# proger/haloop

Measured on AMD Instinct MI355X. Metric: utterances/sec, LSTM-CTC training step (fwd + CTC loss + bwd + clip + AdamW), higher is better.
Workload: dtype bf16 (dense operands rounded to bf16, 1 MFMA per product, fp32 accumulate; fp32 state, CTC, optimizer and master weights); 1 GPU; LC-2x1024: conv(80->128,k5,s4) + 2-layer LSTM H=1024 + Linear(1024->32) + CTC, 80 frames x 80 mels, vocab 32, targets 5-10 symbols, dropout 0.2; batch_per_gpu=64, global_batch=64, frames=80, mels=80, parallelism=dp1, hip_graph=False, math=bf16

## Files before the change

haloop_amd/_lib.py:

```python
import ctypes as C
import os

_HERE = os.path.dirname(os.path.abspath(__file__))
LIB_PATH = os.path.join(_HERE, 'csrc', 'libhalo.so')

HALO_ABI_VERSION = 19
HALO_GEMM_RELU = 1
HALO_GEMM_GELU = 2
HALO_GEMM_ACCUM = 4
HALO_GEMM_GELU_ERF = 8
HALO_CTC_FULL_LATTICE = 1
HALO_CTC_FINITE_MIN = 2
HALO_CTC_NO_LEAD_BLANK_LOOP = 4
HALO_CTC_WRAP_SKIP = 8
HALO_STREAM_SUBSAMPLE = 1
HALO_STREAM_CLASSIFIER = 2
HALO_STREAM_LSTM_LAYER0 = 16
HALO_SUMSQ_PARTS = 1024
HALO_MATH_F32 = 0
HALO_MATH_BF16X3 = 1
HALO_MATH_BF16 = 2

_vp, _i, _l, _f, _u64, _u32, _sz = C.c_void_p, C.c_int, C.c_long, C.c_float, C.c_uint64, C.c_uint32, C.c_size_t

SIGNATURES = {
    'halo_abi_version': (_i, []),
    'halo_debug_read': (_i, [_vp, _sz, _i, _sz, _vp, _vp]),
    'halo_strerror': (C.c_char_p, [_i]),
    'halo_device_info': (_i, [_i, C.c_char_p, _i, C.POINTER(_i)]),
    'halo_set_math_mode': (_i, [_i]),
    'halo_get_math_mode': (_i, []),
    'halo_set_scratch': (_i, [_vp, _sz]),
    'halo_set_lstm_fusion': (_i, [_i]),
    'halo_dropout_fwd': (_i, [_vp, _vp, _sz, _f, _u64, _u32, _u32, _vp, _vp]),
    'halo_counter_inc': (_i, [_vp, _vp]),
    'halo_gemm_f32': (_i, [_i, _i, _i, _i, _i, _vp, _i, _vp, _i, _vp, _i, _vp, _vp, _i, _f, _u64, _u32, _u32, _vp, _vp]),
    'halo_split_image_bytes': (_sz, [_i, _i]),
    'halo_split_image': (_i, [_vp, _i, _i, _i, _i, _vp, _vp]),
    'halo_layernorm_image': (_i, [_vp, _vp, _vp, _vp, _vp, _i, _i, _f, _vp]),
    'halo_layernorm_bf16': (_i, [_vp, _vp, _vp, _vp, _vp, _vp, _i, _i, _f, _vp]),
    'halo_cast_bf16': (_i, [_vp, _vp, _sz, _vp]),
    'halo_gelu_bf16': (_i, [_vp, _vp, _sz, _i, _vp]),
    'halo_gelu_bwd_bf16': (_i, [_vp, _vp, _vp, _sz, _i, _vp]),
    'halo_gemm_tn_bf16_group': (_i, [_i, _vp, _vp, _vp, _vp, _vp, _vp, _i, _vp, _vp, _i, _vp]),
    'halo_gemm_tn_rows_supported': (_i, [_i, _vp, _vp, _i]),
    'halo_gemm_tn_rows_preferred': (_i, [_i, _vp, _vp, _i]),
    'halo_gemm_tn_rows_group': (_i, [_i, _vp, _vp, _vp, _vp, _vp, _vp, _i, _vp, _vp, _vp]),
    'halo_gelu_b16': (_i, [_vp, _vp, _sz, _i, _vp]),
    'halo_gelu_bwd_b16': (_i, [_vp, _vp, _vp, _sz, _i, _vp]),
    'halo_dx_alloc': (_i, [_sz, _vp, _vp]),
    'halo_dx_open': (_i, [_vp, _vp]),
    'halo_dx_close': (_i, [_vp]),
    'halo_dx_free': (_i, [_vp]),
    'halo_dx_push': (_i, [_vp, _sz, _sz, _i, _vp, _sz, _i, _i, _vp]),
    'halo_dx_signal': (_i, [_vp, _sz, _i, _i, _u32, _vp]),
    'halo_dx_wait': (_i, [_vp, _i, _i, _u32, _vp]),
    'halo_dx_reduce': (_i, [_vp, _vp, _sz, _i, _i, _f, _vp]),
    'halo_attention_fwd_b16': (_i, [_vp, _l, _l, _vp, _vp, _l, _l, _vp, _l, _l, _vp, _l, _l, _vp, _i, _i, _i, _i, _i, _i, _vp]),
    'halo_attention_bwd_b16': (_i, [_vp, _l, _l, _vp, _vp, _l, _l, _vp, _vp, _l, _l, _vp, _vp, _vp, _vp, _vp, _l, _l, _i, _i, _i, _i, _i, _i, _vp]),
    'halo_gemm_rows_supported': (_i, [_i, _i, _i]),
    'halo_gemm_rows': (_i, [_vp, _vp, _l, _vp, _i, _i, _i, _vp, _l, _vp, _l, _vp, _l, _vp]),
    'halo_gemm_rows_gelu': (_i, [_vp, _vp, _l, _vp, _i, _i, _i, _vp, _vp, _l, _i, _vp]),
    'halo_gemm_rows_ce_workspace_bytes': (_sz, [_i, _i]),
    'halo_gemm_rows_ce': (_i, [_vp, _vp, _l, _vp, _i, _i, _i, _vp, _l, _vp, _vp, _vp, _vp, _l, _vp]),
    'halo_cross_entropy_bwd_bf16': (_i, [_vp, _vp, _vp, _vp, _l, _i, _i, _l, _l, _vp]),
    'halo_gemm_split_ce_workspace_bytes': (_sz, [_i, _i]),
    'halo_gemm_split_ce': (_i, [_vp, _vp, _i, _i, _i, _vp, _i, _vp, _vp, _l, _vp, _vp, _vp, _vp]),
    'halo_image_pair': (_i, [_vp, _vp, _i, _i, _l, _l, _i, _vp, _vp, _vp]),
    'halo_cross_entropy_bwd_images': (_i, [_vp, _vp, _vp, _vp, _l, _i, _i, _l, _l, _vp, _vp, _vp]),
    'halo_gemm_split': (_i, [_vp, _vp, _i, _i, _i, _vp, _i, _vp, _vp, _i, _f, _u64, _u32, _u32, _vp, _vp]),
    'halo_gemm_split_residual': (_i, [_vp, _vp, _i, _i, _i, _vp, _i, _vp, _i, _vp, _vp, _i, _f, _u64, _u32, _u32, _vp, _vp]),
    'halo_image_pairs': (_i, [_i, _vp, _vp, _vp, _vp, _vp, _vp, _vp]),
    'halo_gemm_split_io': (_i, [_vp, _vp, _vp, _l, _vp, _i, _i, _i, _vp, _i, _vp, _vp, _l, _vp, _i, _vp, _vp, _i, _vp]),
    'halo_gemm_tn_bf16': (_i, [_vp, _l, _vp, _l, _i, _i, _i, _vp, _i, _i, _vp]),
    'halo_subsample_col_bytes': (_sz, [_i] * 6),
    'halo_subsample_fwd': (_i, [_vp] * 5 + [_i] * 7 + [_f, _u64, _u32, _vp, _vp]),
    'halo_subsample_bwd': (_i, [_vp] * 6 + [_i] * 7 + [_f, _vp]),
    'halo_subsample_bwd_slabs': (_i, [_vp, _i] + [_vp] * 5 + [_i] * 7 + [_f, _vp]),
    'halo_lstm_reserve_bytes': (_sz, [_i] * 5),
    'halo_lstm_bwd_workspace_bytes': (_sz, [_i] * 5),
    'halo_lstm_fwd': (_i, [_vp] * 8 + [_l, _l, _i, _vp, _vp, _vp] + [_i] * 5 + [_f, _u64, _u32, _vp, _vp]),
    'halo_lstm_bwd': (_i, [_vp] * 4 + [_l, _l, _i] + [_vp] * 9 + [_i] * 7 + [_f, _u64, _u32, _vp, _vp]),
    'halo_set_lstm_persistent': (_i, [_i]),
    'halo_set_lstm_persistent_images': (_i, [_i]),
    'halo_lstm_persistent_eligible': (_i, [_i, _i]),
    'halo_set_lstm_persistent2': (_i, [_i]),
    'halo_set_lstm_interleave': (_i, [_i]),
    'halo_set_gemm256': (_i, [_i]),
    'halo_set_lstm_bwd_mid_event': (_i, [_vp]),
    'halo_lstm_bwd_mid_event_recorded': (_i, []),
    'halo_set_lstm_expect_backward': (_i, [_i]),
    'halo_set_lstm_dx_slabs': (_i, [_i]),
    'halo_set_defer_small_jobs': (_i, [_i]),
    'halo_set_grad_sumsq': (_i, [_vp, _i]),
    'halo_grad_sumsq_state': (_i, [_vp, _vp]),
    'halo_flush_small_jobs': (_i, [_vp]),
    'halo_lstm_dx_slabs_left': (_i, []),
    'halo_set_lstm_weights_stamp': (_i, [_u64]),
    'halo_lstm_persistent2_eligible': (_i, [_i, _i, _i, _i]),
    'halo_lstm_status_offset': (_sz, [_i] * 6),
    'halo_lstm_persist_stamps': (_i, [_vp]),
    'halo_lstm_chain_events': (_i, [_vp, _vp]),
    'halo_lstm_chain_info': (_i, [_i, C.POINTER(_i), C.c_char_p, _i]),
    'halo_log_softmax_fwd': (_i, [_vp, _vp, _i, _i, _vp]),
    'halo_log_softmax_bwd': (_i, [_vp, _vp, _vp, _i, _i, _vp]),
    'halo_colsum': (_i, [_vp, _i, _i, _i, _vp, _vp]),
    'halo_ctc_fwd': (_i, [_vp, _l, _l, _i, _i, _i, _vp, _l, _i, _vp, _vp, _i, _vp, _vp, _vp]),
    'halo_ctc_bwd': (_i, [_vp, _l, _l, _i, _i, _i, _vp, _l, _i, _vp, _vp, _vp, _vp, _vp, _vp, _vp, _l, _l, _vp]),
    'halo_ctc_prepare': (_i, [_vp, _vp, _i, _i, _i, _i, _vp, _vp, _vp]),
    'halo_ctc_mean_loss': (_i, [_vp, _vp, _i, _vp, _vp]),
    'halo_ctc_head_supported': (_i, [_i, _i, _i, _i]),
    'halo_ctc_head_greedy': (_i, [_vp, _vp, _vp, _vp, _vp, _vp, _vp, _vp, _i, _i, _i, _i, _vp]),
    'halo_ctc_head_workspace_bytes': (_sz, [_i, _i, _i]),
    'halo_ctc_head_fwd': (_i, [_vp, _vp, _vp, _f, _u64, _u32, _u32, _vp, _vp, _i, _i, _i, _vp, _l, _i, _vp, _vp, _vp, _vp, _vp, _vp, _vp,
                               _vp, _i, _i, _i, _i, _vp]),
    'halo_ctc_head_bwd': (_i, [_vp, _vp, _f, _u64, _u32, _u32, _vp, _vp, _vp, _l, _i, _vp, _vp, _vp, _vp, _vp, _vp, _vp, _vp, _vp,
                               _i, _i, _i, _i, _vp]),
    'halo_ctc_head_train_workspace_bytes': (_sz, [_i, _i, _i]),
    'halo_ctc_head_train_ticket_words': (_sz, [_i, _i]),
    'halo_ctc_head_train': (_i, [_vp, _vp, _vp, _f, _u64, _u32, _u32, _vp, _vp, _i, _i, _i, _vp, _l, _i, _vp, _vp, _vp, _vp, _vp, _vp, _vp,
                                 _vp, _vp, _vp, _i, _i, _i, _i, _vp]),
    'halo_ctc_greedy': (_i, [_vp, _i, _i, _i, _vp, _vp, _vp, _vp, _vp]),
    'halo_set_beam_vector_chunk': (_i, [_i]),
    'halo_logaddexp_aten': (_i, [_vp, _vp, _vp, _sz, _vp]),
    'halo_ctc_beam_workspace_bytes': (_sz, [_i] * 4),
    'halo_ctc_beam': (_i, [_vp, _i, _i, _i, _i, _i, _vp, _vp, _vp, _vp, _vp]),
    'halo_topk_f32': (_i, [_vp, _i, _i, _i, _vp, _vp, _vp, _vp]),
    'halo_embed_fwd': (_i, [_vp, _vp, _vp, _vp, _i, _i, _i, _i, _i, _vp]),
    'halo_layernorm_fwd': (_i, [_vp, _vp, _vp, _vp, _i, _i, _f, _vp]),
    'halo_attention_causal_fwd': (_i, [_vp, _vp, _i, _i, _i, _i, _vp]),
    'halo_cross_entropy_fwd': (_i, [_vp, _vp, _vp, _i, _i, _l, _l, _vp]),
    'halo_attention_fwd': (_i, [_vp, _l, _l, _vp, _vp, _l, _l, _vp, _l, _l, _vp, _vp, _i, _i, _i, _i, _i, _i, _vp, _vp]),
    'halo_attention_fwd_strided': (_i, [_vp, _l, _l, _l, _vp, _vp, _l, _l, _l, _vp, _l, _l, _vp, _vp, _i, _i, _i, _i, _i, _i, _vp,
                                        _f, _u64, _u32, _u32, _vp, _vp]),
    'halo_kv_cache_store_f32': (_i, [_vp, _l, _l, _vp, _vp, _i, _i, _i, _i, _i, _i, _vp]),
    'halo_rope_table': (_i, [_vp, _vp, _i, _i, _f, _vp]),
    'halo_rope_interleaved': (_i, [_vp, _l, _i, _i, _i, _i, _i, _vp, _vp, _i, _i, _vp]),
    'halo_kv_cache_store': (_i, [_vp, _l, _l, _vp, _vp, _i, _i, _i, _i, _i, _i, _vp]),
    'halo_attention_decode': (_i, [_vp, _l, _vp, _vp, _vp, _l, _i, _i, _i, _i, _i, _vp, _vp, _vp, _vp]),
    'halo_attention_decode_step': (_i, [_vp, _vp, _vp, _l, _vp, _vp, _vp, _l, _i, _i, _i, _i, _i, _vp, _vp, _vp]),
    'halo_logprob_max': (_i, [_vp, _l, _i, _i, _vp, _vp, _vp, _vp]),
    'halo_greedy_update': (_i, [_vp, _vp, _vp, _vp, _l, _i, _i, _i, _vp, _vp, _vp, _vp, _i, _vp]),
    'halo_fbank_frames': (_i, [_vp, _l, _i, _i, _i, _f, _i, _vp, _vp, _i, _vp]),
    'halo_fbank_power': (_i, [_vp, _i, _i, _vp, _i, _vp]),
    'halo_fbank_log': (_i, [_vp, _l, _f, _vp]),
    'halo_fbank_spectrum_mel': (_i, [_vp, _i, _i, _vp, _vp, _i, _f, _vp, _vp]),
    'halo_star_ctc_workspace_bytes': (_sz, [_i, _i, _i]),
    'halo_star_ctc_fwd': (_i, [_vp, _l, _l, _i, _i, _i, _vp, _i, _vp, _vp, _f, _vp, _vp, _vp]),
    'halo_star_ctc_bwd': (_i, [_vp, _l, _l, _i, _i, _i, _vp, _i, _vp, _vp, _f, _vp, _vp, _vp, _vp, _vp]),
    'halo_transducer_workspace_bytes': (_sz, [_i, _i, _i]),
    'halo_transducer_fwd': (_i, [_vp, _i, _i, _i, _i, _vp, _vp, _vp, _vp, _vp, _vp]),
    'halo_transducer_bwd': (_i, [_vp, _i, _i, _i, _i, _vp, _vp, _vp, _vp, _vp, _vp, _vp, _vp]),
    'halo_decode_image_bytes': (_sz, [_i, _i]),
    'halo_decode_image': (_i, [_vp, _i, _i, _l, _vp, _vp]),
    'halo_decode_linear_supported': (_i, [_i, _i]),
    'halo_decode_linear': (_i, [_vp, _l, _i, _i, _vp, _f, _vp, _i, _vp, _l, _i, _vp]),
    'halo_decode_linear_pair': (_i, [_vp, _vp, _l, _i, _i, _vp, _f, _vp, _i, _vp, _vp, _vp, _l, _i, _vp]),
    'halo_decode_attention_pair': (_i, [_vp, _l, _i, _i, _i, _vp, _vp, _i, _vp, _vp, _vp, _i, _i, _vp, _vp, _vp, _l, _vp]),
    'halo_decode_memory_caches': (_i, [_vp, _l, _i, _vp, _i, _i, _i, _i, _vp]),
    'halo_decode_token': (_i, [_vp, _l, _i, _i, _vp, _l, _i, _i, _i, _vp, _vp, _vp, _vp, _vp, _i, _i, _vp, _vp]),
    'halo_attention_bwd': (_i, [_vp, _l, _l, _vp, _vp, _l, _l, _vp, _vp, _l, _l, _vp, _vp, _vp, _l, _l, _vp, _vp, _l, _l,
                                _i, _i, _i, _i, _i, _i, _vp, _f, _u64, _u32, _u32, _vp, _vp]),
    'halo_attention_masked': (_i, [_vp, _vp, _vp, _vp, _l, _l, _l, _vp, _vp, _i, _i, _i, _i, _i, _vp]),
    'halo_attention_fwd_bf16': (_i, [_vp, _l, _l, _vp, _vp, _l, _l, _vp, _l, _l, _vp, _l, _l, _vp, _i, _i, _i, _i, _i, _i, _vp, _f, _u64, _u32, _u32,
                                     _vp, _vp]),
    'halo_attention_bwd_bf16': (_i, [_vp, _l, _l, _vp, _vp, _l, _l, _vp, _vp, _l, _l, _vp, _vp, _vp, _vp, _vp, _l, _l, _i, _i, _i, _i, _i, _i, _vp,
                                     _f, _u64, _u32, _u32, _vp, _vp]),
    'halo_layernorm_bwd_workspace_bytes': (_sz, [_i, _i]),
    'halo_layernorm_bwd': (_i, [_vp, _vp, _vp, _vp, _vp, _vp, _vp, _vp, _i, _i, _f, _vp]),
    'halo_layernorm_bwd_bf16': (_i, [_vp, _vp, _vp, _vp, _vp, _vp, _vp, _vp, _vp, _i, _i, _f, _vp]),
    'halo_layernorm_bwd_b16': (_i, [_vp, _vp, _vp, _vp, _vp, _vp, _vp, _vp, _vp, _i, _i, _f, _vp]),
    'halo_gelu_fwd': (_i, [_vp, _vp, _sz, _i, _vp]),
    'halo_gelu_bwd': (_i, [_vp, _vp, _vp, _sz, _i, _vp]),
    'halo_cross_entropy_fwd_lse': (_i, [_vp, _vp, _vp, _vp, _i, _i, _l, _l, _vp]),
    'halo_cross_entropy_bwd': (_i, [_vp, _vp, _vp, _vp, _l, _i, _i, _l, _l, _vp]),
    'halo_embed_bwd': (_i, [_vp, _vp, _vp, _vp, _i, _i, _i, _i, _i, _i, _vp]),
    'halo_add_rows_bcast': (_i, [_vp, _vp, _i, _i, _i, _vp]),
    'halo_im2col_cl': (_i, [_vp, _vp, _i, _i, _i, _i, _i, _i, _vp]),
    'halo_col2im_cl': (_i, [_vp, _vp, _i, _i, _i, _i, _i, _i, _vp]),
    'halo_dwconv1d_cl': (_i, [_vp, _vp, _vp, _vp, _i, _i, _i, _i, _i, _i, _vp]),
    'halo_dwconv1d_cl_bwd_workspace_bytes': (_sz, [_i, _i]),
    'halo_dwconv1d_cl_bwd': (_i, [_vp, _vp, _vp, _vp, _vp, _vp, _vp, _i, _i, _i, _i, _i, _i, _vp]),
    'halo_tape_batch': (_i, [_vp, _i, _l, _i, _i, _l, _i, _l, _vp, _vp]),
    'halo_lm_batch_u16': (_i, [_vp, _l, _vp, _i, _i, _i, _vp, _vp, _vp]),
    'halo_scale_add': (_i, [_vp, _vp, _f, _f, _sz, _vp]),
    'halo_cast_f32_bf16': (_i, [_vp, _vp, _sz, _vp]),
    'halo_cast_bf16_f32': (_i, [_vp, _vp, _f, _sz, _vp]),
    'halo_scale_add_guarded': (_i, [_vp, _vp, _f, _f, _sz, _vp, _vp]),
    'halo_clip_coef_step': (_i, [_vp, _i, _f, _vp, _vp, _vp, _vp]),
    'halo_adamw_ranges_dev': (_i, [_vp, _vp, _vp, _vp, _i, _vp, _vp, _vp, _vp, _f, _vp, _f, _f, _f, _vp, _vp, _vp]),
    'halo_ctx_create': (_vp, []),
    'halo_ctx_destroy': (None, [_vp]),
    'halo_ctx_use': (_i, [_vp]),
    'halo_set_status_word': (_i, [_vp]),
    'halo_debug_mute_workgroup': (_i, [_i]),
    'halo_debug_mfma_clock': (_i, [_vp, _vp, _i, _i, _i, _u32, _vp]),
    'halo_sumsq': (_i, [_vp, _sz, _vp, _vp]),
    'halo_sumsq_ranges': (_i, [_vp, _i, _vp, _vp, _vp, _vp]),
    'halo_pack_ranges_bf16': (_i, [_vp, _i, _vp, _vp, _vp, _vp]),
    'halo_expand_ranges_bf16': (_i, [_vp, _i, _vp, _vp, _i, _i, _vp, _vp]),
    'halo_clip_coef': (_i, [_vp, _i, _f, _vp, _vp, _vp]),
    'halo_adamw_multi_tensor_bytes': (_sz, []),
    'halo_adamw_multi_chunk': (_u32, []),
    'halo_adamw_multi_max_tensors': (_i, []),
    'halo_adamw_multi': (_i, [_vp, _vp, _i, _vp, _i, _f, _f, _f, _f, _i, _vp, _vp]),
    'halo_adamw_ranges': (_i, [_vp, _vp, _vp, _vp, _i, _vp, _vp, _vp, _vp, _f, _f, _f, _f, _i, _vp, _vp]),
    'halo_adamw': (_i, [_vp, _vp, _vp, _vp, _sz, _f, _f, _f, _f, _f, _i, _vp, _vp]),
}

_lib = None


class HaloError(RuntimeError):
    pass


def lib():
    global _lib
    if _lib is None:
        import torch
        if not os.path.exists(LIB_PATH):
            raise HaloError(f'{LIB_PATH} not found: build it with `make -C haloop_amd/csrc` '
                            '(or __graft_entry__.build()); haloop_amd has no CPU fallback')
        handle = C.CDLL(LIB_PATH)
        for name, (res, args) in SIGNATURES.items():
            fn = getattr(handle, name)
            fn.restype = res
            fn.argtypes = args
        if handle.halo_abi_version() != HALO_ABI_VERSION:
            raise HaloError('libhalo.so ABI version mismatch: rebuild it')
        _lib = handle
        mode = os.environ.get('HALO_MATH')
        if mode:
            set_math_mode(mode)
    return _lib


def set_math_mode(mode):
    global _mode
    code = {'f32': HALO_MATH_F32, 'bf16x3': HALO_MATH_BF16X3, 'bf16': HALO_MATH_BF16}[mode]
    check(lib().halo_set_math_mode(code), 'halo_set_math_mode')
    _mode = mode


def set_lstm_fusion(on):
    check(lib().halo_set_lstm_fusion(int(bool(on))), 'halo_set_lstm_fusion')


def set_lstm_persistent(on):
    check(lib().halo_set_lstm_persistent(int(bool(on))), 'halo_set_lstm_persistent')


def set_lstm_bwd_mid_event(event):
    check(lib().halo_set_lstm_bwd_mid_event(None if event is None else C.c_void_p(event.cuda_event)), 'halo_set_lstm_bwd_mid_event')


def set_gemm256(on):
    check(lib().halo_set_gemm256(1 if on else 0), 'halo_set_gemm256')


def set_lstm_interleave(on):
    check(lib().halo_set_lstm_interleave(int(bool(on))), 'halo_set_lstm_interleave')


def set_lstm_persistent2(on):
    check(lib().halo_set_lstm_persistent2(int(bool(on))), 'halo_set_lstm_persistent2')


_WEIGHTS_EPOCH = [0]


def bump_weights_epoch():
    _WEIGHTS_EPOCH[0] += 1
# ... 105 lines not shown
```

haloop_amd/csrc/halo_internal.h:

```cpp
#pragma once
#include <hip/hip_runtime.h>
#include <stddef.h>
#include "halo_common.h"
#include "small_jobs.h"

int halo_transpose(const float *in, float *out, int rows, int cols, hipStream_t st);
int halo_fill(float *p, size_t n, float v, hipStream_t st);
int halo_colsum2(const float *x, int rows, int cols, int ld, float *out, float *out2, hipStream_t st);

size_t halo_tiled_image_bytes(int R, int K);
int halo_prep_tiles(const float *src, int R, int K, int ld, int src_transposed, void *image, hipStream_t st);
int halo_prep_pair(const float *src, int R, int C, int ld, void *image_rm, void *image_tr, hipStream_t st);
struct HaloPrepJob {
    int kind;
    const float *src;
    int R, K, ld;
    void *image, *image_tr;
};
int halo_prep_jobs(const HaloPrepJob *jobs, int n, hipStream_t st);
int halo_gemm_bf16x3_tiled(const void *Aimg, const void *Bimg, int M, int N, int K, float *C, int ldc,
                           const float *bias1, const float *bias2, int relu, const DropoutCfg *drop, hipStream_t st);
int halo_gemm_bf16x3_tiled_slices(const void *Aimg, const void *Bimg, int M, int N, int K, float *slab, int want, int *slices, hipStream_t st);
bool halo_defer_small_job(const HaloSmallJob &job);
struct HaloCtx {
    int math_mode = 0;
    int lstm_fusion = 0;
    int lstm_persistent = 1, lstm_persistent2 = 1;
    int lstm_interleave = 1;
    int persist_emit = -1;
    int beam_vec_chunk = 32;
    void *scratch = nullptr;
    size_t scratch_bytes = 0;
    int scratch_slot = 0;
    unsigned *status = nullptr;
    hipEvent_t chain_ev0 = nullptr, chain_ev1 = nullptr;
    int bwd_mid_recorded = 0;
    hipEvent_t bwd_mid_event = nullptr;
    unsigned long long *stamps = nullptr;
    float *grad_sumsq = nullptr;
    int grad_sumsq_cap = 0, grad_sumsq_n = 0;
    unsigned grad_sumsq_cover = 0;
    int defer_small_jobs = 0;
    HaloSmallJobs small_jobs = {};
    int lstm_dx_slabs = 1;
    int lstm_dx_slabs_left = 1;
    int lstm_expect_backward = 1;
    const float *packT_reserve = nullptr, *packT_w[3] = {nullptr, nullptr, nullptr};
    const float *bwdflags_reserve = nullptr;
    const float *fwdT_src[2] = {nullptr, nullptr};
    const float *fwdT_reserve = nullptr;
    const float *emitT_reserve = nullptr;
    uint64_t lstm_weights_stamp = 0, packF_stamp = 0;
    const float *packF_reserve = nullptr, *packF_w[3] = {nullptr, nullptr, nullptr};
    int packF_dims[5] = {0, 0, 0, 0, 0};
    int mute_block = -1;
};
HaloCtx &halo_ctx_cur();
int halo_cu_count();
bool halo_func_attr_done(int slot);
void halo_func_attr_set(int slot);
int halo_gemm_bf16x3_tiled_nsplit(const void *Aimg, const void *Bimg, int M, int N, int K, float *C, int ldc, int n_split, float *C2, int ldc2,
                                  hipStream_t st);
int halo_gemm_bf16x3_tiled_nsplit_carry(const void *Aimg, const void *Bimg, int M, int N, int K, float *C, int ldc, int n_split, float *C2, int ldc2,
                                        const void *rA, const void *rB, int rM, int rN, int rK, float *rslab, int want, int *slices,
                                        float *sumsq_part, int *sumsq_parts, hipStream_t st);
struct HaloG256Problem {
    const void *A, *B;
    int M, N, K;
    float *C; int ldc;
    int n_split; float *C2; int ldc2;
    int kslices; long slab_stride;
    float *sumsq;
    int tiles;
};
int halo_gemm256_enabled();
int halo_gemm256_fits(const HaloG256Problem &q);
int halo_gemm256_launch(HaloG256Problem *probs, int n, hipStream_t st);
int halo_math_mode();
int halo_lstm_fusion();

void halo_get_scratch(void **ptr, size_t *bytes);
void halo_set_scratch_slot(int slot);
int halo_side_stream(hipStream_t *side, hipEvent_t *fork_ev, hipEvent_t *join_ev);
int halo_pick_ksplit(long tiles, int k_steps, long out_elems);
int halo_splitk_reduce(const float *slab, int ksplit, int M, int N, float *C, int ldc, const float *bias1,
                       const float *bias2, int relu, const DropoutCfg &drop, int use_drop, hipStream_t st);
```

haloop_amd/csrc/lstm.hip:

```cpp
#include <stdlib.h>
#include <string.h>
#include "halo_common.h"
#include "halo_internal.h"
#include "tiled_image.h"
#include "lstm_persist.h"

namespace {

enum YMode { Y_NONE = 0, Y_PLAIN = 1, Y_RELU = 2, Y_DROPOUT = 3 };

typedef __bf16 bf16x8 __attribute__((ext_vector_type(8)));

template <bool X3>
struct Packed {
    static constexpr int KB = X3 ? 32 : 16;
    static constexpr int BLOCK_BYTES = X3 ? 2048 : 1024;
    __device__ static __forceinline__ void store(void *img, int tile, int nk, int i, int k, float v) {
        const int blk = k / KB, kk = k % KB;
        char *base = (char *)img + ((long)tile * (nk / KB) + blk) * BLOCK_BYTES;
        if (X3) {
            const int lane = (kk >> 3) * 16 + i, e = kk & 7;
            const __bf16 hi = (__bf16)v;
            const __bf16 lo = (__bf16)(v - (float)hi);
            reinterpret_cast<__bf16 *>(base)[lane * 8 + e] = hi;
// ... 1115 lines not shown

inline bool keep_dg_switch() {
    static const bool on = getenv("HALO_LSTM_KEEP_DG") && getenv("HALO_LSTM_KEEP_DG")[0] == '1';
    return on;
}

inline bool pair_dw_enabled() {
    static const bool on = !(getenv("HALO_LSTM_PAIR_DW") && atoi(getenv("HALO_LSTM_PAIR_DW")) == 0);
    return on;
}

int lstm_bwd_layer_tail(const float *x, const float *const *w_ih, float *reserve, int l, int in0, int T, int B, int H, int L, float p_drop,
                        uint64_t seed, uint32_t offset, const uint32_t *offset_dev, bool fused, bool emit, char *img_g, char *img_gT,
                        char *img_hT, char *img_inT, char *img_wT, const float *bias_part, float *din, float *dx, float *const *dw_ih,
                        float *const *dw_hh, float *const *db_ih, float *const *db_hh, bool need_din, hipStream_t st) {
    const size_t BH = (size_t)B * H;
    const LayerBufs lb = layer_bufs(reserve, l, T, B, H);
    hipStream_t side = st;
    const float *in;
    int in_dim;
    if (l == 0) { in = x; in_dim = in0; }
    else {
        const LayerBufs pb = layer_bufs(reserve, l - 1, T, B, H);
        in = p_drop > 0.f ? pb.ydrop : pb.h + BH;
        in_dim = H;
    }
    (void)fused;
    float *din_out = l > 0 ? din : dx;
    const DropoutCfg ddrop = make_dropout(l > 0 ? p_drop : 0.f, seed, HALO_STREAM_LSTM_LAYER0 + (uint32_t)(l > 0 ? l - 1 : 0),
                                          offset, offset_dev);
    const bool tiled = halo_math_mode() != HALO_MATH_F32 && in_dim >= 64;
    int rc = HALO_OK;
    if (tiled) {
        HaloPrepJob jobs[5];
        int nj = 0;
        if (need_din) {
            if (!emit) jobs[nj++] = {2, lb.gates, T * B, 4 * H, 4 * H, img_g, img_gT};
            jobs[nj++] = {1, w_ih[l], in_dim, 4 * H, in_dim, img_wT, nullptr};
        } else if (!emit) {
            jobs[nj++] = {1, lb.gates, 4 * H, T * B, 4 * H, img_gT, nullptr};
        }
        if (emit)
            jobs[nj++] = {3, bias_part, (B + 15) / 16, 4 * H, 4 * H, db_ih[l], db_hh[l]};
        jobs[nj++] = {1, lb.h, H, T * B, H, img_hT, nullptr};
        jobs[nj++] = {1, in, in_dim, T * B, in_dim, img_inT, nullptr};
        HALO_TRY(halo_prep_jobs(jobs, nj, st));
    }
    if (need_din) {
        if (tiled) {
            HALO_TRY(halo_gemm_bf16x3_tiled(img_g, img_wT, T * B, in_dim, 4 * H, din_out, in_dim, nullptr, nullptr, 0,
                                            &ddrop, st));
        } else {
            HALO_TRY(halo_gemm_f32(1, 0, T * B, in_dim, 4 * H, lb.gates, 4 * H, w_ih[l], in_dim, din_out, in_dim,
                                   nullptr, nullptr, 0, l > 0 ? p_drop : 0.f, seed,
                                   HALO_STREAM_LSTM_LAYER0 + (uint32_t)(l > 0 ? l - 1 : 0), offset, offset_dev, (halo_stream_t)st));
        }
    }
    if (tiled && H % 128 == 0 && img_inT == img_hT + halo_tiled_image_bytes(H, T * B) && pair_dw_enabled()) {
        HaloG256Problem gp = {};
        gp.A = img_gT; gp.B = img_hT; gp.M = 4 * H; gp.N = H + in_dim; gp.K = T * B;
        gp.C = dw_hh[l]; gp.ldc = H; gp.n_split = H; gp.C2 = dw_ih[l]; gp.ldc2 = in_dim; gp.kslices = 1;
        const long t256 = (long)((4 * H + 255) / 256) * ((H + in_dim + 255) / 256);
        if (halo_gemm256_enabled() && halo_gemm256_fits(gp) && 100 * t256 >= 55 * ((t256 + 255) / 256) * 256) rc = halo_gemm256_launch(&gp, 1, side);
        else
        rc = halo_gemm_bf16x3_tiled_nsplit(img_gT, img_hT, 4 * H, H + in_dim, T * B, dw_hh[l], H, H, dw_ih[l], in_dim, side);
    } else if (tiled) {
        rc = halo_gemm_bf16x3_tiled(img_gT, img_hT, 4 * H, H, T * B, dw_hh[l], H, nullptr, nullptr, 0, nullptr, side);
        if (!rc) rc = halo_gemm_bf16x3_tiled(img_gT, img_inT, 4 * H, in_dim, T * B, dw_ih[l], in_dim, nullptr, nullptr, 0,
                                             nullptr, side);
    } else {
        rc = halo_gemm_f32(0, 0, 4 * H, H, T * B, lb.gates, 4 * H, lb.h, H, dw_hh[l], H, nullptr, nullptr, 0, 0.f, 0, 0,
                           0, nullptr, (halo_stream_t)side);
        if (!rc) rc = halo_gemm_f32(0, 0, 4 * H, in_dim, T * B, lb.gates, 4 * H, in, in_dim, dw_ih[l], in_dim, nullptr,
                                    nullptr, 0, 0.f, 0, 0, 0, nullptr, (halo_stream_t)side);
    }
    if (!rc && !(emit && tiled)) rc = halo_colsum2(lb.gates, T * B, 4 * H, 4 * H, db_ih[l], db_hh[l], side);
    return rc;
}


int lstm_fwd_persist2(const float *in, int in_dim, int lo, const float *const *w_ih, const float *const *w_hh, const float *const *b_ih,
                      const float *const *b_hh, const float *h0, const float *c0, float *y, long y_stride_t, long y_stride_b,
                      int y_relu, float *hn, float *cn, float *reserve, float *extra, char *img_in, char *img_w, int T, int B,
                      int in0, int H, int L, float p_drop, uint64_t seed, uint32_t offset, const uint32_t *offset_dev, hipStream_t st) {
    const int hi = lo + 1;
    const size_t BH = (size_t)B * H;
    const LayerBufs l0 = layer_bufs(reserve, lo, T, B, H), l1 = layer_bufs(reserve, hi, T, B, H);
    w_ih += lo; w_hh += lo; b_ih += lo; b_hh += lo;
    if (h0) h0 += (size_t)lo * BH;
    if (c0) c0 += (size_t)lo * BH;
    HaloCtx &ctx = halo_ctx_cur();
    const bool images_by_pack = in_dim >= 64;
    if (in_dim < 64) {
        HALO_TRY(halo_gemm_f32(1, 1, T * B, 4 * H, in_dim, in, in_dim, w_ih[0], in_dim, l0.gates, 4 * H, b_ih[0], b_hh[0], 0, 0.f, 0, 0, 0,
                               nullptr, (halo_stream_t)st));
    }
    float *wp0 = reserve, *wp1 = fused_wpk(extra, hi, H), *wpi = wp1 + (size_t)4 * H * H;
    unsigned *flags = (unsigned *)((char *)reserve + reserve_flags_offset(T, B, in0, H, L));
    Prologue2Args pa;
    pa.img.n = 0; pa.img.blocks = 0; pa.img.with_lo = halo_math_mode() != HALO_MATH_BF16;
    pa.w[0] = w_hh[0]; pa.wdst[0] = wp0; pa.w[1] = w_hh[1]; pa.wdst[1] = wp1; pa.w[2] = w_ih[1]; pa.wdst[2] = wpi;
    pa.w_units = (long)(H / 16) * 4 * (H / 32) * 64; pa.wK = H;
    for (int l = 0; l < 2; ++l) {
        const LayerBufs lb = l ? l1 : l0;
        pa.h0[l] = h0 ? h0 + (size_t)l * BH : nullptr; pa.hp0[l] = lb.hp; pa.h_rm[l] = lb.h;
        pa.c0[l] = c0 ? c0 + (size_t)l * BH : nullptr; pa.c_rm[l] = lb.c;
    }
    pa.s_units = (long)((B + 15) / 16) * (H / 32) * 64;
    pa.zero = flags; pa.zero_units = (long)(PERSIST_FLAG_BYTES / 16);
    pa.zero2 = nullptr; pa.zero2_units = 0;
    char *xp = p_drop > 0.f ? (char *)fused_yp(extra, lo, T, B, H, L) : nullptr;
    pa.narm = 0; pa.arm_units = 0;
    if (halo_lstm_persist2_fwd_armed(T, B, H)) {
        const size_t image = (size_t)((B + 15) / 16) * (H / 32) * 2048;
        pa.arm[pa.narm++] = (char *)l0.hp + image;
        pa.arm[pa.narm++] = (char *)l1.hp + image;
        if (xp) pa.arm[pa.narm++] = xp;
        pa.arm_units = (long)T * (long)(image / 2048) * 64;
    }
    pa.H = H; pa.B = B;
    ctx.packT_reserve = nullptr;
    ctx.emitT_reserve = nullptr;
    char *emit_hT0 = nullptr, *emit_hT1 = nullptr, *emit_xT1 = nullptr;
    if (ctx.lstm_expect_backward && H % 32 == 0) {
        float *wT = (float *)((char *)reserve + reserve_flags_offset(T, B, in0, H, L) + PERSIST_FLAG_BYTES);
        PackPairArgs pp;
        for (int m = 0; m < 3; ++m) { pp.w[m] = pa.w[m]; pp.fwd[m] = (char *)pa.wdst[m]; pp.tr[m] = (char *)(wT + (size_t)m * 4 * H * H); }
        pp.H = H;
        pp.tile_blocks = 3 * (4 * H / 32) * (H / 32) / 4;
        pp.rest = pa; pp.rest.w_units = 0;
        pp.rest.zero2 = reserve_bwd_flags(reserve, T, B, in0, H, L); pp.rest.zero2_units = (long)(PERSIST_FLAG_BYTES / 16);
        pp.zbase[0] = pp.zbase[1] = nullptr; pp.zstride = 0; pp.zunits = 0; pp.zcount = 0;
        ctx.emitT_reserve = nullptr;
        const bool emitT = persist_emit_enabled() && !h0 && B % 32 == 0 && H % 128 == 0 && T * B >= 32;
        if (emitT) {
            char *imgs = reserve_p2_images(reserve, T, B, in0, H, L);
            const size_t hb = halo_tiled_image_bytes(H, T * B), ib = halo_tiled_image_bytes(in0 > H ? in0 : H, T * B);
            emit_hT0 = imgs; emit_hT1 = imgs + hb + ib; emit_xT1 = emit_hT1 + hb;
            const long KT = (T * B + 31) / 32;
            pp.zbase[0] = emit_hT0; pp.zbase[1] = emit_hT1;
            pp.zstride = KT * 16384; pp.zunits = (long)(B / 32) * 16384 / 16; pp.zcount = H / 128;
            ctx.emitT_reserve = reserve;
        }
        ctx.fwdT_reserve = nullptr;
        if (images_by_pack) {
            ImageJobs &ij = pp.rest.img;
            image_jobs_add(ij, in, T * B, in_dim, in_dim, 0, img_in);
            image_jobs_add(ij, w_ih[0], 4 * H, in_dim, in_dim, 0, img_w);
            if (emitT) {
                image_jobs_add(ij, in, in_dim, T * B, in_dim, 1, emit_hT0 + halo_tiled_image_bytes(H, T * B));
                image_jobs_add(ij, w_ih[0], in_dim, 4 * H, in_dim, 1, reserve_p2_wT(reserve, T, B, in0, H, L));
                ctx.fwdT_reserve = reserve; ctx.fwdT_src[0] = in; ctx.fwdT_src[1] = w_ih[0];
            }
        }
        const unsigned rest_blocks = pack_grid((size_t)(2 * pa.s_units + pa.zero_units + pp.rest.zero2_units + 2L * pp.zcount * pp.zunits +
                                                        (long)pa.narm * pa.arm_units));
        hipLaunchKernelGGL(persist2_pack_pair_kernel, dim3((unsigned)(pp.tile_blocks + pp.rest.img.blocks) + rest_blocks), dim3(256), 0, st, pp);
        HALO_TRY(halo_launch_status());
        if (images_by_pack)
            HALO_TRY(halo_gemm_bf16x3_tiled(img_in, img_w, T * B, 4 * H, in_dim, l0.gates, 4 * H, b_ih[0], b_hh[0], 0, nullptr, st));
        ctx.packT_reserve = reserve;
        ctx.bwdflags_reserve = reserve;
        for (int m = 0; m < 3; ++m) ctx.packT_w[m] = pa.w[m];
    } else {
        const int dims[5] = {T, B, in0, H, L};
        const bool keep = ctx.lstm_weights_stamp != 0 && lo == 0 && ctx.packF_stamp == ctx.lstm_weights_stamp && ctx.packF_reserve == reserve &&
                          ctx.packF_w[0] == pa.w[0] && ctx.packF_w[1] == pa.w[1] && ctx.packF_w[2] == pa.w[2] &&
                          !memcmp(ctx.packF_dims, dims, sizeof(dims));
        if (keep) pa.w_units = 0;
        if (images_by_pack) {
            image_jobs_add(pa.img, in, T * B, in_dim, in_dim, 0, img_in);
            image_jobs_add(pa.img, w_ih[0], 4 * H, in_dim, in_dim, 0, img_w);
        }
        hipLaunchKernelGGL(persist2_prologue_kernel<0>, dim3((unsigned)pa.img.blocks + pack_grid((size_t)(3 * pa.w_units + 2 * pa.s_units + pa.zero_units +
                                                                                                      (long)pa.narm * pa.arm_units))),
                           dim3(256), 0, st, pa);
        HALO_TRY(halo_launch_status());
        if (images_by_pack)
            HALO_TRY(halo_gemm_bf16x3_tiled(img_in, img_w, T * B, 4 * H, in_dim, l0.gates, 4 * H, b_ih[0], b_hh[0], 0, nullptr, st));
        ctx.packF_stamp = lo == 0 ? ctx.lstm_weights_stamp : 0;
        ctx.packF_reserve = reserve;
        for (int m = 0; m < 3; ++m) ctx.packF_w[m] = pa.w[m];
        memcpy(ctx.packF_dims, dims, sizeof(dims));
    }
    Persist2Fwd a;
    a.wp0 = (const char *)wp0; a.wp1 = (const char *)wp1; a.wpi = (const char *)wpi;
    a.hp0 = (char *)l0.hp; a.hp1 = (char *)l1.hp;
    a.xp = xp;
    a.gates0 = l0.gates; a.h0 = l0.h; a.c0 = l0.c;
    a.gates1 = l1.gates; a.h1 = l1.h; a.c1 = l1.c;
    a.b_ih1 = b_ih[1]; a.b_hh1 = b_hh[1];
    a.ydrop = p_drop > 0.f ? l0.ydrop : nullptr;
    a.y = y; a.y_stride_t = y_stride_t; a.y_stride_b = y_stride_b; a.y_mode = y ? (y_relu ? 2 : 1) : 0;
    a.drop = make_dropout(p_drop, seed, HALO_STREAM_LSTM_LAYER0 + (uint32_t)lo, offset, offset_dev);
    a.img_hT0 = emit_hT0; a.img_hT1 = emit_hT1; a.img_xT1 = emit_xT1;
    a.flags = flags;
    a.stamps = halo_lstm_persist_stamp_buffer();
    a.T = T; a.B = B; a.H = H;
    chain_begin(st);
    HALO_TRY(halo_lstm_persist2_fwd(a, st));
    chain_end(st, 0, 1, "lstm_persist2_fwd_kernel");
    for (int l = 0; l < 2; ++l) {
        const LayerBufs lb = l ? l1 : l0;
        if (hn) HALO_TRY(copy_d2d(hn + (size_t)(lo + l) * BH, lb.h + (size_t)T * BH, BH, st));
        if (cn) HALO_TRY(copy_d2d(cn + (size_t)(lo + l) * BH, lb.c + (size_t)T * BH, BH, st));
    }
    return HALO_OK;
}


inline size_t bwd_p2_offset(int T, int B, int in0, int H, int L) {
    const size_t n = bwd_flags_offset(T, B, in0, H, L) + PERSIST_FLAG_BYTES + (size_t)((B + 15) / 16) * 4 * H * sizeof(float);
// ... 3 lines not shown
    return (((size_t)((B + 15) / 16) * 4 * H * sizeof(float) + 255) & ~(size_t)255) + (size_t)T * bt16(B) * 4 * H * sizeof(float) +
           halo_tiled_image_bytes(4 * H, T * B);
}

}

extern "C" {

int halo_lstm_chain_events(void *ev_begin, void *ev_end) {
    halo_ctx_cur().chain_ev0 = (hipEvent_t)ev_begin;
    halo_ctx_cur().chain_ev1 = (hipEvent_t)ev_end;
    return HALO_OK;
}

int halo_lstm_chain_info(int backward, int *launches, char *kernel, int kernel_len) {
    const ChainInfo &ci = g_chain_info[backward ? 1 : 0];
    if (launches) *launches = ci.launches;
    if (kernel && kernel_len > 0) {
        strncpy(kernel, ci.kernel, (size_t)kernel_len - 1);
        kernel[kernel_len - 1] = 0;
    }
    return HALO_OK;
}

size_t halo_lstm_reserve_bytes(int T, int B, int in0, int H, int L) {
    if (T <= 0 || B <= 0 || in0 <= 0 || H <= 0 || L <= 0) return 0;
    return reserve_flags_offset(T, B, in0, H, L) + PERSIST_FLAG_BYTES + (L >= 2 ? reserve_p2_bytes(T, B, in0, H) : 0);
}

int halo_set_lstm_persistent(int on) {
    halo_lstm_persist_enable(on);
    return HALO_OK;
}

int halo_set_lstm_persistent_images(int on) {
    halo_ctx_cur().persist_emit = on ? 1 : 0;
    return HALO_OK;
}


int halo_lstm_persistent_eligible(int B, int H) { return halo_lstm_persist_ok(B, H) && use_x3(H) ? 1 : 0; }

int halo_set_lstm_persistent2(int on) {
    halo_lstm_persist2_enable(on);
    return HALO_OK;
}
int halo_set_lstm_bwd_mid_event(void *event) {
    halo_ctx_cur().bwd_mid_event = (hipEvent_t)event;
    halo_ctx_cur().bwd_mid_recorded = 0;
    return HALO_OK;
}
int halo_lstm_bwd_mid_event_recorded(void) { return halo_ctx_cur().bwd_mid_recorded; }
int halo_set_lstm_interleave(int on) {
    halo_lstm_interleave_enable(on);
    return HALO_OK;
}
int halo_set_lstm_weights_stamp(uint64_t stamp) {
    halo_ctx_cur().lstm_weights_stamp = stamp;
    return HALO_OK;
}

int halo_set_grad_sumsq(float *partials, int capacity) {
    HaloCtx &ctx = halo_ctx_cur();
    if (partials && capacity <= 0) return HALO_EINVAL;
    ctx.grad_sumsq = partials; ctx.grad_sumsq_cap = partials ? capacity : 0; ctx.grad_sumsq_n = 0; ctx.grad_sumsq_cover = 0;
    return HALO_OK;
}
int halo_grad_sumsq_state(int *count, unsigned *covered) {
    const HaloCtx &ctx = halo_ctx_cur();
    if (count) *count = ctx.grad_sumsq_n;
    if (covered) *covered = ctx.grad_sumsq_cover;
    return HALO_OK;
}
int halo_set_lstm_dx_slabs(int n) {
    if (n < 1 || n > 64) return HALO_EINVAL;
    halo_ctx_cur().lstm_dx_slabs = n;
    return HALO_OK;
}
int halo_lstm_dx_slabs_left(void) { return halo_ctx_cur().lstm_dx_slabs_left; }
int halo_set_lstm_expect_backward(int on) {
    halo_ctx_cur().lstm_expect_backward = on ? 1 : 0;
    return HALO_OK;
}
int halo_lstm_persistent2_eligible(int T, int B, int H, int L) {       return !fused_ok(H, L) && use_x3(H) && halo_lstm_persist2_ok(T, B, H, L) ? 1 : 0; }

size_t halo_lstm_status_offset(int backward, int T, int B, int in0, int H, int L) {
    if (T <= 0 || B <= 0 || in0 <= 0 || H <= 0 || L <= 0) return 0;
    return backward ? bwd_flags_offset(T, B, in0, H, L) : reserve_flags_offset(T, B, in0, H, L);
}

size_t halo_lstm_bwd_workspace_bytes(int T, int B, int in0, int H, int L) {
    if (T <= 0 || B <= 0 || H <= 0 || L <= 0) return 0;
    if (L >= 2) return bwd_p2_offset(T, B, in0, H, L) + bwd_p2_bytes(T, B, H);
    return bwd_flags_offset(T, B, in0, H, L) + PERSIST_FLAG_BYTES + (size_t)((B + 15) / 16) * 4 * H * sizeof(float);
}

int halo_lstm_fwd(const float *x, const float *const *w_ih, const float *const *w_hh, const float *const *b_ih,
                  const float *const *b_hh, const float *h0, const float *c0, float *y, long y_stride_t,
                  long y_stride_b, int y_relu, float *hn, float *cn, float *reserve, int T, int B, int in0, int H,
                  int L, float p_drop, uint64_t seed, uint32_t offset, const uint32_t *offset_dev,
                  halo_stream_t stream) {
    HALO_CHECK_ARG(x && w_ih && w_hh && b_ih && b_hh && reserve);
    HALO_CHECK_ARG(T > 0 && B > 0 && in0 > 0 && H > 0 && L > 0);
    if (H % 16 != 0) return HALO_ENOTSUP;
    hipStream_t st = (hipStream_t)stream;
    const size_t BH = (size_t)B * H, PH = bt16(B) * H;
    halo_ctx_cur().packT_reserve = nullptr;
    halo_ctx_cur().emitT_reserve = nullptr;
    float *wp = reserve;
    const bool x3 = use_x3(H);
    const int kin = in0 > H ? in0 : H;
    char *img_in = (char *)(reserve + (size_t)4 * H * H + (size_t)L * layer_floats(T, B, H));
    char *img_w = img_in + halo_tiled_image_bytes(T * B, kin);
    for (int l = 0; l < L; ++l) HALO_CHECK_ARG(w_ih[l] && w_hh[l] && b_ih[l] && b_hh[l]);
    const bool pair = !fused_ok(H, L) && x3 && halo_lstm_persist2_ok(T, B, H, L);
    const int n_single = pair ? L - 2 : L;
    if (fused_ok(H, L)) {
        float *extra = (float *)(img_w + halo_tiled_image_bytes(4 * H, kin));
        return lstm_fwd_fused(x, w_ih, w_hh, b_ih, b_hh, h0, c0, y, y_stride_t, y_stride_b, y_relu, hn, cn, reserve, extra,
                              img_in, img_w, T, B, in0, H, L, p_drop, seed, offset, offset_dev, st);
    }
    for (int l = 0; l < L; ++l) {
        const LayerBufs lb = layer_bufs(reserve, l, T, B, H);
        const bool last = (l == L - 1);
        const bool drop_out = !last && p_drop > 0.f;
        const float *in;
        int in_dim;
        if (l == 0) { in = x; in_dim = in0; }
        else {
            const LayerBufs pb = layer_bufs(reserve, l - 1, T, B, H);
            in = p_drop > 0.f ? pb.ydrop : pb.h + BH;
            in_dim = H;
        }
        if (pair && l == n_single) {
            float *extra = (float *)(img_w + halo_tiled_image_bytes(4 * H, kin));
            return lstm_fwd_persist2(in, in_dim, l, w_ih, w_hh, b_ih, b_hh, h0, c0, y, y_stride_t, y_stride_b, y_relu, hn, cn, reserve, extra,
                                     img_in, img_w, T, B, in0, H, L, p_drop, seed, offset, offset_dev, st);
        }
        if (halo_math_mode() != HALO_MATH_F32 && in_dim >= 64) {
            const HaloPrepJob jobs[2] = {{0, in, T * B, in_dim, in_dim, img_in, nullptr}, {0, w_ih[l], 4 * H, in_dim, in_dim, img_w, nullptr}};
            HALO_TRY(halo_prep_jobs(jobs, 2, st));
            HALO_TRY(halo_gemm_bf16x3_tiled(img_in, img_w, T * B, 4 * H, in_dim, lb.gates, 4 * H, b_ih[l], b_hh[l], 0,
                                            nullptr, st));
        } else {
            HALO_TRY(halo_gemm_f32(1, 1, T * B, 4 * H, in_dim, in, in_dim, w_ih[l], in_dim, lb.gates, 4 * H, b_ih[l],
                                   b_hh[l], 0, 0.f, 0, 0, 0, nullptr, stream));
        }
        const float *h0l = h0 ? h0 + (size_t)l * BH : nullptr;
        const bool persist = x3 && halo_lstm_persist_ok(B, H) && halo_lstm_persist_fits(T, B, H);
        unsigned *flags = (unsigned *)((char *)reserve + reserve_flags_offset(T, B, in0, H, L));
        if (persist) {
            PrologueArgs pa;
            pa.w = w_hh[l]; pa.wdst = wp; pa.w_units = (long)(H / 16) * 4 * (H / 32) * 64; pa.wK = H;
            pa.h0 = h0l; pa.hp0 = lb.hp; pa.h_rm = lb.h; pa.c0 = c0 ? c0 + (size_t)l * BH : nullptr; pa.c_rm = lb.c;
            pa.s_units = (long)((B + 15) / 16) * (H / 32) * 64;
            pa.zero = flags; pa.zero_units = (long)(PERSIST_FLAG_BYTES / 16);
            pa.zero2 = nullptr; pa.zero2_units = 0;
            pa.H = H; pa.B = B;
            hipLaunchKernelGGL(persist_prologue_kernel<0>, dim3(pack_grid((size_t)(pa.w_units + pa.s_units + pa.zero_units))), dim3(256), 0, st, pa);
            HALO_TRY(halo_launch_status());
        } else {
            HALO_TRY(launch_pack<0>(w_hh[l], wp, H, B, H, (H / 16) * 4, x3, st));
            HALO_TRY(launch_pack<2>(h0l, lb.hp, H, B, H, (B + 15) / 16, x3, st, lb.h, c0 ? c0 + (size_t)l * BH : nullptr, lb.c));
        }
        const DropoutCfg dc = make_dropout(drop_out ? p_drop : 0.f, seed, HALO_STREAM_LSTM_LAYER0 + (uint32_t)l, offset, offset_dev);
        if (persist) {
            PersistFwd a;
            a.wp = (const char *)wp;
            a.hp = (char *)lb.hp;
            a.gates = lb.gates; a.h = lb.h; a.c = lb.c;
            a.T = T; a.B = B; a.H = H;
            a.drop = dc;
            if (last && y) { a.y = y; a.y_stride_t = y_stride_t; a.y_stride_b = y_stride_b; a.y_mode = y_relu ? Y_RELU : Y_PLAIN; }
            else if (drop_out) { a.y = lb.ydrop; a.y_stride_t = (long)BH; a.y_stride_b = H; a.y_mode = Y_DROPOUT; }
            else { a.y = nullptr; a.y_stride_t = 0; a.y_stride_b = 0; a.y_mode = Y_NONE; }
            a.flags = flags;
            a.stamps = halo_lstm_persist_stamp_buffer();
            chain_begin(st);
            HALO_TRY(halo_lstm_persist_fwd(a, st));
            chain_end(st, 0, 1, "lstm_persist_fwd_kernel");
            if (hn) HALO_TRY(copy_d2d(hn + (size_t)l * BH, lb.h + (size_t)T * BH, BH, st));
            if (cn) HALO_TRY(copy_d2d(cn + (size_t)l * BH, lb.c + (size_t)T * BH, BH, st));
            continue;
        }
        chain_begin(st);
        for (int t = 0; t < T; ++t) {
            StepFwdArgs a;
            a.hp_prev = lb.hp + (size_t)t * PH;
            a.cprev = lb.c + (size_t)t * BH;
            a.wp = wp;
            a.gates = lb.gates + (size_t)t * B * 4 * H;
            a.hout = lb.h + (size_t)(t + 1) * BH;
            a.hp_out = lb.hp + (size_t)(t + 1) * PH;
            a.cout = lb.c + (size_t)(t + 1) * BH;
            a.B = B; a.H = H;
            a.drop = dc;
            a.drop_base = (uint64_t)t * BH;
            if (last && y) {
                a.y = y + (long)t * y_stride_t;
                a.y_stride_b = y_stride_b;
                a.y_mode = y_relu ? Y_RELU : Y_PLAIN;
            } else if (drop_out) {
                a.y = lb.ydrop + (size_t)t * BH;
                a.y_stride_b = H;
                a.y_mode = Y_DROPOUT;
            } else {
                a.y = nullptr; a.y_stride_b = 0; a.y_mode = Y_NONE;
            }
            HALO_TRY(launch_step_fwd(a, x3, st));
        }
        chain_end(st, 0, T, "lstm_step_fwd_kernel");
        if (hn) HALO_TRY(copy_d2d(hn + (size_t)l * BH, lb.h + (size_t)T * BH, BH, st));
        if (cn) HALO_TRY(copy_d2d(cn + (size_t)l * BH, lb.c + (size_t)T * BH, BH, st));
    }
    return HALO_OK;
}

int halo_lstm_bwd(const float *x, const float *const *w_ih, const float *const *w_hh, const float *dy,
                  long y_stride_t, long y_stride_b, int y_relu, const float *dhn, const float *dcn, float *reserve,
                  float *workspace, float *dx, float *const *dw_ih, float *const *dw_hh, float *const *db_ih,
// ... 265 lines not shown
```

haloop_amd/csrc/optim.hip:

```cpp
#include <math.h>
#include <stdlib.h>
#include "halo_common.h"
#include "halo_internal.h"

namespace {

__global__ __launch_bounds__(256) void sumsq_kernel(const float *__restrict__ x, size_t n, float *__restrict__ partials) {
    __shared__ float red[4];
    float s = 0.f;
    const size_t n4 = n / 4;
    const f32x4 *x4 = reinterpret_cast<const f32x4 *>(x);
    for (size_t i = blockIdx.x * (size_t)256 + threadIdx.x; i < n4; i += (size_t)gridDim.x * 256) {
        const f32x4 v = x4[i];
        s += v[0] * v[0] + v[1] * v[1] + v[2] * v[2] + v[3] * v[3];
    }
    if (blockIdx.x == 0)
        for (size_t i = n4 * 4 + threadIdx.x; i < n; i += 256) s += x[i] * x[i];
    s = wave_sum(s);
    if ((threadIdx.x & 63) == 0) red[threadIdx.x >> 6] = s;
    __syncthreads();
    if (threadIdx.x == 0) partials[blockIdx.x] = (red[0] + red[1]) + (red[2] + red[3]);
}

struct Ranges8 {
// ... 98 lines not shown
    float bc2_sqrt;
    float eps;
    const float *grad_scale;
};

__global__ __launch_bounds__(256) void adamw_kernel(const AdamArgs a) {
    const float gs = a.grad_scale ? *a.grad_scale : 1.0f;
    if (gs != gs) return;
    const size_t n4 = a.n / 4;
    f32x4 *p4 = reinterpret_cast<f32x4 *>(a.p), *m4 = reinterpret_cast<f32x4 *>(a.m), *v4 = reinterpret_cast<f32x4 *>(a.v);
    const f32x4 *g4 = reinterpret_cast<const f32x4 *>(a.g);
    for (size_t i = blockIdx.x * (size_t)256 + threadIdx.x; i < n4; i += (size_t)gridDim.x * 256) {
        f32x4 p = p4[i], m = m4[i], v = v4[i];
        const f32x4 g = g4[i];
#pragma unroll
        for (int e = 0; e < 4; ++e) {
            const float ge = a.grad_scale ? g[e] * gs : g[e];
            float pe = p[e], me = m[e], ve = v[e];
            adam_update(pe, me, ve, ge, a.decay_mul, a.beta1_w, a.beta2, a.beta2_w, a.step_size, a.bc2_sqrt, a.eps);
            p[e] = pe; m[e] = me; v[e] = ve;
        }
        p4[i] = p; m4[i] = m; v4[i] = v;
    }
    if (blockIdx.x == 0) {
        for (size_t i = n4 * 4 + threadIdx.x; i < a.n; i += 256) {
            const float ge = a.grad_scale ? a.g[i] * gs : a.g[i];
            float pe = a.p[i], me = a.m[i], ve = a.v[i];
            adam_update(pe, me, ve, ge, a.decay_mul, a.beta1_w, a.beta2, a.beta2_w, a.step_size, a.bc2_sqrt, a.eps);
            a.p[i] = pe; a.m[i] = me; a.v[i] = ve;
        }
    }
}


constexpr int ADAM_MAX_RANGES = 8;
struct AdamRangesArgs {
    float *p;
    const float *g;
    float *m;
    float *v;
    size_t begin4[ADAM_MAX_RANGES], end4[ADAM_MAX_RANGES];
    float decay_mul[ADAM_MAX_RANGES];
    const float *grad_scale[ADAM_MAX_RANGES];
    int n_ranges;
    float beta1_w, beta2, beta2_w, step_size, bc2_sqrt, eps;
    uint32_t *counter;
    const uint32_t *step_dev;
    const float *lr_dev;
    float weight_decay[ADAM_MAX_RANGES];
    float lr, beta1;
};

template <bool NT>
__global__ __launch_bounds__(256) void adamw_ranges_kernel(const AdamRangesArgs a) {
    f32x4 *p4 = reinterpret_cast<f32x4 *>(a.p), *m4 = reinterpret_cast<f32x4 *>(a.m), *v4 = reinterpret_cast<f32x4 *>(a.v);
    const f32x4 *g4 = reinterpret_cast<const f32x4 *>(a.g);
    float step_size = a.step_size, bc2_sqrt = a.bc2_sqrt;
    const float lr = a.lr_dev ? *a.lr_dev : a.lr;
    if (a.step_dev) {
        const double t = (double)max(*a.step_dev, 1u);
        step_size = (float)((double)lr / (1.0 - pow((double)a.beta1, t)));
        bc2_sqrt = (float)sqrt(1.0 - pow((double)a.beta2, t));
    }
    for (int r = 0; r < a.n_ranges; ++r) {
        const float gs = a.grad_scale[r] ? *a.grad_scale[r] : 1.0f;
        if (gs != gs) continue;
        const float decay_mul = a.lr_dev ? (float)(1.0 - (double)lr * (double)a.weight_decay[r]) : a.decay_mul[r];
        for (size_t i = a.begin4[r] + blockIdx.x * (size_t)256 + threadIdx.x; i < a.end4[r]; i += (size_t)gridDim.x * 256) {
            f32x4 p = p4[i], m = NT ? __builtin_nontemporal_load(m4 + i) : m4[i], v = NT ? __builtin_nontemporal_load(v4 + i) : v4[i];
            const f32x4 g = NT ? __builtin_nontemporal_load(g4 + i) : g4[i];
#pragma unroll
            for (int e = 0; e < 4; ++e) {
                const float ge = a.grad_scale[r] ? g[e] * gs : g[e];
                float pe = p[e], me = m[e], ve = v[e];
                adam_update(pe, me, ve, ge, decay_mul, a.beta1_w, a.beta2, a.beta2_w, step_size, bc2_sqrt, a.eps);
                p[e] = pe; m[e] = me; v[e] = ve;
            }
            p4[i] = p;
            if (NT) { __builtin_nontemporal_store(m, m4 + i); __builtin_nontemporal_store(v, v4 + i); }
            else { m4[i] = m; v4[i] = v; }
        }
    }
    if (a.counter && blockIdx.x == 0 && threadIdx.x == 0) *a.counter += 1u;
}

struct AdamTensor {
    float *p;
    float *m;
    float *v;
    unsigned long long n;
    float weight_decay;
    int pad;
};
constexpr unsigned ADAM_CHUNK = 16384;
constexpr int ADAM_MULTI_MAX = 256;
struct AdamGrads { const float *g[ADAM_MULTI_MAX]; };

__global__ __launch_bounds__(256) void adamw_multi_kernel(const AdamTensor *__restrict__ tensors, const uint2 *__restrict__ chunks,
                                                          const AdamGrads grads, float lr, float beta1_w, float beta2, float beta2_w,
                                                          float step_size, float bc2_sqrt, float eps,
                                                          const float *__restrict__ grad_scale) {
    const float gs = grad_scale ? *grad_scale : 1.0f;
    if (gs != gs) return;
    const uint2 c = chunks[blockIdx.x];
    const AdamTensor t = tensors[c.x];
    const float decay_mul = (float)(1.0 - (double)lr * (double)t.weight_decay);
    const float *tg = grads.g[c.x];
    const size_t begin = (size_t)c.y * ADAM_CHUNK, end = min(begin + (size_t)ADAM_CHUNK, (size_t)t.n);
    auto update = [&](float &pe, float &me, float &ve, float g) {
        adam_update(pe, me, ve, grad_scale ? g * gs : g, decay_mul, beta1_w, beta2, beta2_w, step_size, bc2_sqrt, eps);
    };
    const bool vec = (((uintptr_t)t.p | (uintptr_t)tg | (uintptr_t)t.m | (uintptr_t)t.v) % 16) == 0;
    size_t done = begin;
    if (vec) {
        const size_t e4 = end / 4;
        f32x4 *p4 = reinterpret_cast<f32x4 *>(t.p), *m4 = reinterpret_cast<f32x4 *>(t.m), *v4 = reinterpret_cast<f32x4 *>(t.v);
        const f32x4 *g4 = reinterpret_cast<const f32x4 *>(tg);
        for (size_t i = begin / 4 + threadIdx.x; i < e4; i += 256) {
            f32x4 p = p4[i], m = __builtin_nontemporal_load(m4 + i), v = __builtin_nontemporal_load(v4 + i);
            const f32x4 g = __builtin_nontemporal_load(g4 + i);
#pragma unroll
            for (int e = 0; e < 4; ++e) {
                float pe = p[e], me = m[e], ve = v[e];
                update(pe, me, ve, g[e]);
                p[e] = pe; m[e] = me; v[e] = ve;
            }
            p4[i] = p;
            __builtin_nontemporal_store(m, m4 + i);
            __builtin_nontemporal_store(v, v4 + i);
        }
        done = e4 * 4;
    }
    for (size_t i = done + threadIdx.x; i < end; i += 256) {
        float pe = t.p[i], me = t.m[i], ve = t.v[i];
        update(pe, me, ve, tg[i]);
        t.p[i] = pe; t.m[i] = me; t.v[i] = ve;
    }
}

}

namespace {
__global__ __launch_bounds__(256) void scale_add_kernel(float *__restrict__ y, const float *__restrict__ x, float alpha, float beta, size_t n4,
                                                        size_t n, const float *__restrict__ guard) {
    const size_t i = (size_t)blockIdx.x * 256 + threadIdx.x;
    const bool take_x = !guard || isfinite(*guard);
    const bool take_y = alpha != 0.f;
    if (i < n4) {
        f32x4 a = {0.f, 0.f, 0.f, 0.f}, b = {0.f, 0.f, 0.f, 0.f};
        if (take_y) a = alpha * reinterpret_cast<f32x4 *>(y)[i];
        if (take_x) b = beta * reinterpret_cast<const f32x4 *>(x)[i];
        reinterpret_cast<f32x4 *>(y)[i] = a + b;
    } else if (i == n4) {
        for (size_t e = 4 * n4; e < n; ++e) y[e] = (take_y ? alpha * y[e] : 0.f) + (take_x ? beta * x[e] : 0.f);
    }
}
}

namespace {
typedef __bf16 bf16x4 __attribute__((ext_vector_type(4)));
__global__ __launch_bounds__(256) void cast_f32_bf16_kernel(const float *__restrict__ x, __bf16 *__restrict__ y, size_t n4, size_t n) {
    for (size_t i = (size_t)blockIdx.x * 256 + threadIdx.x; i < n4; i += (size_t)gridDim.x * 256) {
        const f32x4 v = reinterpret_cast<const f32x4 *>(x)[i];
        bf16x4 o;
#pragma unroll
        for (int e = 0; e < 4; ++e) o[e] = (__bf16)v[e];
// ... 114 lines not shown
}

int halo_adamw(float *p, const float *g, float *m, float *v, size_t n, float lr, float beta1, float beta2, float eps,
               float weight_decay, int step, const float *grad_scale, halo_stream_t stream) {
    HALO_CHECK_ARG(p && g && m && v && step >= 1);
    HALO_CHECK_ARG(((uintptr_t)p % 16 == 0) && ((uintptr_t)g % 16 == 0) && ((uintptr_t)m % 16 == 0) &&
                   ((uintptr_t)v % 16 == 0));
    if (n == 0) return HALO_OK;
    AdamArgs a;
    a.p = p; a.g = g; a.m = m; a.v = v; a.n = n;
    const double bc1 = 1.0 - pow((double)beta1, (double)step);
    const double bc2 = 1.0 - pow((double)beta2, (double)step);
    a.decay_mul = (float)(1.0 - (double)lr * (double)weight_decay);
    a.beta1_w = (float)(1.0 - (double)beta1);
    a.beta2 = beta2;
    a.beta2_w = (float)(1.0 - (double)beta2);
    a.step_size = (float)((double)lr / bc1);
    a.bc2_sqrt = (float)sqrt(bc2);
    a.eps = eps;
    a.grad_scale = grad_scale;
    size_t blocks = (n / 4 + 255) / 256;
    if (blocks < 1) blocks = 1;
    if (blocks > 2048) blocks = 2048;
    hipLaunchKernelGGL(adamw_kernel, dim3((unsigned)blocks), dim3(256), 0, (hipStream_t)stream, a);
    return halo_launch_status();
}

size_t halo_adamw_multi_tensor_bytes(void) { return sizeof(AdamTensor); }
unsigned halo_adamw_multi_chunk(void) { return ADAM_CHUNK; }

int halo_adamw_multi_max_tensors(void) { return ADAM_MULTI_MAX; }

int halo_adamw_multi(const void *tensor_table, const void *chunk_table, int n_chunks, const float *const *grads, int n_tensors, float lr,
                     float beta1, float beta2, float eps, int step, const float *grad_scale, halo_stream_t stream) {
    HALO_CHECK_ARG(tensor_table && chunk_table && n_chunks > 0 && step >= 1 && grads && n_tensors > 0 && n_tensors <= ADAM_MULTI_MAX);
    AdamGrads gr;
    for (int i = 0; i < ADAM_MULTI_MAX; ++i) gr.g[i] = i < n_tensors ? grads[i] : nullptr;
    for (int i = 0; i < n_tensors; ++i) HALO_CHECK_ARG(grads[i] != nullptr);
    const double bc1 = 1.0 - pow((double)beta1, (double)step);
    const double bc2 = 1.0 - pow((double)beta2, (double)step);
    hipLaunchKernelGGL(adamw_multi_kernel, dim3((unsigned)n_chunks), dim3(256), 0, (hipStream_t)stream, (const AdamTensor *)tensor_table,
                       (const uint2 *)chunk_table, gr, lr, (float)(1.0 - (double)beta1), beta2, (float)(1.0 - (double)beta2),
                       (float)((double)lr / bc1), (float)sqrt(bc2), eps, grad_scale);
    return halo_launch_status();
}

static int adamw_ranges_impl(float *p, const float *g, float *m, float *v, int n_ranges, const size_t *begin, const size_t *end,
                      const float *weight_decay, const float *const *grad_scale, float lr, float beta1, float beta2, float eps, int step,
                      const uint32_t *step_dev, const float *lr_dev, uint32_t *counter, halo_stream_t stream) {
    HALO_CHECK_ARG(p && g && m && v && begin && end && weight_decay && grad_scale && n_ranges > 0 && n_ranges <= ADAM_MAX_RANGES &&
                   (step >= 1 || step_dev) && (!lr_dev || step_dev));
    HALO_CHECK_ARG(((uintptr_t)p % 16 == 0) && ((uintptr_t)g % 16 == 0) && ((uintptr_t)m % 16 == 0) && ((uintptr_t)v % 16 == 0));
    AdamRangesArgs a;
    a.p = p; a.g = g; a.m = m; a.v = v; a.n_ranges = n_ranges; a.counter = counter;
    a.step_dev = step_dev; a.lr_dev = lr_dev; a.lr = lr; a.beta1 = beta1;
    if (step < 1) step = 1;
    size_t biggest = 0;
    for (int r = 0; r < n_ranges; ++r) {
        HALO_CHECK_ARG(begin[r] % 4 == 0 && end[r] % 4 == 0 && begin[r] <= end[r]);
        a.begin4[r] = begin[r] / 4; a.end4[r] = end[r] / 4;
        a.decay_mul[r] = (float)(1.0 - (double)lr * (double)weight_decay[r]);
        a.weight_decay[r] = weight_decay[r];
        a.grad_scale[r] = grad_scale[r];
        if (a.end4[r] - a.begin4[r] > biggest) biggest = a.end4[r] - a.begin4[r];
    }
    const double bc1 = 1.0 - pow((double)beta1, (double)step);
    const double bc2 = 1.0 - pow((double)beta2, (double)step);
    a.beta1_w = (float)(1.0 - (double)beta1);
    a.beta2 = beta2;
    a.beta2_w = (float)(1.0 - (double)beta2);
    a.step_size = (float)((double)lr / bc1);
    a.bc2_sqrt = (float)sqrt(bc2);
    a.eps = eps;
    size_t blocks = (biggest + 255) / 256;
    if (blocks > 4096) blocks = 4096;
    if (blocks < 1) blocks = 1;
    static int nt = -1;
    if (nt < 0) { const char *e = getenv("HALO_ADAMW_NT"); nt = (e && e[0] == '0') ? 0 : 1; }
    if (nt) hipLaunchKernelGGL(adamw_ranges_kernel<true>, dim3((unsigned)blocks), dim3(256), 0, (hipStream_t)stream, a);
    else hipLaunchKernelGGL(adamw_ranges_kernel<false>, dim3((unsigned)blocks), dim3(256), 0, (hipStream_t)stream, a);
    return halo_launch_status();
}

int halo_adamw_ranges(float *p, const float *g, float *m, float *v, int n_ranges, const size_t *begin, const size_t *end,
                      const float *weight_decay, const float *const *grad_scale, float lr, float beta1, float beta2, float eps, int step,
                      uint32_t *counter, halo_stream_t stream) {
    return adamw_ranges_impl(p, g, m, v, n_ranges, begin, end, weight_decay, grad_scale, lr, beta1, beta2, eps, step, nullptr, nullptr,
                             counter, stream);
}

int halo_adamw_ranges_dev(float *p, const float *g, float *m, float *v, int n_ranges, const size_t *begin, const size_t *end,
                          const float *weight_decay, const float *const *grad_scale, float lr, const float *lr_dev, float beta1, float beta2,
                          float eps, const uint32_t *step_dev, uint32_t *counter, halo_stream_t stream) {
    HALO_CHECK_ARG(step_dev);
    return adamw_ranges_impl(p, g, m, v, n_ranges, begin, end, weight_decay, grad_scale, lr, beta1, beta2, eps, 0, step_dev, lr_dev,
                             counter, stream);
}

}
```

haloop_amd/ops.py:

```python
import ctypes as C

import torch

from . import _lib
from ._lib import check, lib, ptr, ptr_array


def _stream():
    return torch._C._cuda_getCurrentRawStream(torch.cuda.current_device())


def _f32c(t, name):
    if t.dtype != torch.float32 or not t.is_cuda or not t.is_contiguous():
        raise ValueError(f'{name}: expected a contiguous float32 HIP tensor, got {t.dtype} {t.device} '
                         f'contiguous={t.is_contiguous()}')
    return t


class Dropout:
    __slots__ = ('p', 'seed', 'offset', 'counter')

    def __init__(self, p=0.0, seed=0, offset=0, counter=None):
        self.p, self.seed, self.offset, self.counter = float(p), int(seed), int(offset), counter

# ... 295 lines not shown
    return y


def gelu_bwd_b16(dy, a, exact=False):
    y = torch.empty_like(a)
    check(lib().halo_gelu_bwd_b16(ptr(dy), ptr(a), ptr(y), a.numel(), int(exact), _stream()), 'halo_gelu_bwd_b16')
    return y


def dropout_fwd(x, drop, stream_id):
    _f32c(x, 'x')
    y = torch.empty_like(x)
    check(lib().halo_dropout_fwd(ptr(x), ptr(y), x.numel(), drop.p, drop.seed, stream_id, drop.offset,
                                 drop.counter_ptr, _stream()), 'halo_dropout_fwd')
    return y


def subsample_fwd(x, w, bias, drop, ks=5, stride=4, pad=3):
    _f32c(x, 'inputs'); _f32c(w, 'subsample.weight'); _f32c(bias, 'subsample.bias')
    B, T, F = x.shape
    Cc = w.shape[0]
    Tp = subsampled_length(T, ks, stride, pad)
    y = torch.empty(Tp, B, Cc, device=x.device, dtype=torch.float32)
    col = torch.empty(Tp * B, F * ks, device=x.device, dtype=torch.float32)
    check(lib().halo_subsample_fwd(ptr(x), ptr(w), ptr(bias), ptr(y), ptr(col), B, T, F, Cc, ks, stride, pad,
                                   drop.p, drop.seed, drop.offset, drop.counter_ptr, _stream()), 'halo_subsample_fwd')
    return y, col


def subsample_bwd(dy, y, col, B, T, F, Cc, p_drop, dw=None, dbias=None, ks=5, stride=4, pad=3, slabs=1):
    _f32c(dy, 'dy')
    if slabs > 1 and dy.numel() < slabs * y.numel():
        raise ValueError('haloop_amd.ops.subsample_bwd: dy holds fewer than `slabs` matrices')
    dpre = torch.empty_like(y)
    if dw is None:
        dw = torch.empty(Cc, F, ks, device=y.device, dtype=torch.float32)
    if dbias is None:
        dbias = torch.empty(Cc, device=y.device, dtype=torch.float32)
    check(lib().halo_subsample_bwd_slabs(ptr(dy), int(slabs), ptr(y), ptr(col), ptr(dpre), ptr(dw), ptr(dbias), B, T, F, Cc, ks, stride,
                                         pad, p_drop, _stream()), 'halo_subsample_bwd_slabs')
    return dw, dbias


def lstm_fwd(x_tm, w_ih, w_hh, b_ih, b_hh, h0=None, c0=None, y=None, y_strides=None, y_relu=False,
             want_state=False, drop=NO_DROPOUT, expect_backward=True, reserve=None, weights_stamp=0):
    _f32c(x_tm, 'x')
    T, B, in0 = x_tm.shape
    L = len(w_hh)
    H = w_hh[0].shape[1]
    for t in list(w_ih) + list(w_hh) + list(b_ih) + list(b_hh):
        _f32c(t, 'lstm parameter')
    dev = x_tm.device
    if y is None:
        y = torch.empty(T, B, H, device=dev, dtype=torch.float32)
        y_strides = (B * H, H)
    need = (lib().halo_lstm_reserve_bytes(T, B, in0, H, L) + 3) // 4
    if reserve is None:
        reserve = torch.empty(need, device=dev, dtype=torch.float32)
    elif reserve.dtype != torch.float32 or reserve.numel() < need or not reserve.is_contiguous():
        raise ValueError('lstm_fwd: the reserve is too small for this shape (ops.lstm_reserve)')
    hn = torch.empty(L, B, H, device=dev, dtype=torch.float32) if want_state else None
    cn = torch.empty(L, B, H, device=dev, dtype=torch.float32) if want_state else None
    if h0 is not None:
        _f32c(h0, 'h0'); _f32c(c0, 'c0')
    a_ih, a_hh, a_bi, a_bh = ptr_array(w_ih), ptr_array(w_hh), ptr_array(b_ih), ptr_array(b_hh)
    if not expect_backward:
        lib().halo_set_lstm_expect_backward(0)
        lib().halo_set_lstm_weights_stamp(int(weights_stamp))
    try:
        check(lib().halo_lstm_fwd(ptr(x_tm), a_ih, a_hh, a_bi, a_bh, ptr(h0), ptr(c0), ptr(y), y_strides[0], y_strides[1],
                                  int(y_relu), ptr(hn), ptr(cn), ptr(reserve), T, B, in0, H, L, drop.p, drop.seed,
                                  drop.offset, drop.counter_ptr, _stream()), 'halo_lstm_fwd')
    finally:
        if not expect_backward:
            lib().halo_set_lstm_expect_backward(1)
            lib().halo_set_lstm_weights_stamp(0)
    return y, hn, cn, reserve


def lstm_reserve(T, B, in0, H, L, device):
    return torch.empty((lib().halo_lstm_reserve_bytes(T, B, in0, H, L) + 3) // 4, device=device, dtype=torch.float32)


def lstm_bwd_workspace(x_tm, w_hh):
    T, B, in0 = x_tm.shape
    return torch.empty((lib().halo_lstm_bwd_workspace_bytes(T, B, in0, w_hh[0].shape[1], len(w_hh)) + 3) // 4,
                       device=x_tm.device, dtype=torch.float32)


def lstm_bwd(x_tm, w_ih, w_hh, dy, y_strides, y_relu, reserve, dhn=None, dcn=None, want_dx=False,
             grads=None, drop=NO_DROPOUT, layers=None, workspace=None, dx=None, dx_slabs=1):
    T, B, in0 = x_tm.shape
    L = len(w_hh)
    H = w_hh[0].shape[1]
    dev = x_tm.device
    if grads is None:
        grads = {
            'dw_ih': [torch.empty_like(w) for w in w_ih],
            'dw_hh': [torch.empty_like(w) for w in w_hh],
            'db_ih': [torch.empty(4 * H, device=dev, dtype=torch.float32) for _ in range(L)],
            'db_hh': [torch.empty(4 * H, device=dev, dtype=torch.float32) for _ in range(L)],
        }
    ws = workspace if workspace is not None else lstm_bwd_workspace(x_tm, w_hh)
    lo, hi = layers if layers is not None else (0, L)
    if dx is None and want_dx and lo == 0:
        dx = torch.empty(T, B, in0, device=dev, dtype=torch.float32)
    a_ih, a_hh = ptr_array(w_ih), ptr_array(w_hh)
    g_ih, g_hh = ptr_array(grads['dw_ih']), ptr_array(grads['dw_hh'])
    g_bi, g_bh = ptr_array(grads['db_ih']), ptr_array(grads['db_hh'])
    if dx_slabs > 1:
        if dx is None or dx.numel() < dx_slabs * T * B * in0:
            raise ValueError('haloop_amd.ops.lstm_bwd: dx_slabs needs a dx buffer of that many [T, B, in] matrices')
        check(lib().halo_set_lstm_dx_slabs(int(dx_slabs)), 'halo_set_lstm_dx_slabs')
    try:
        check(lib().halo_lstm_bwd(ptr(x_tm), a_ih, a_hh, ptr(dy), y_strides[0], y_strides[1], int(y_relu), ptr(dhn),
                                  ptr(dcn), ptr(reserve), ptr(ws), ptr(dx), g_ih, g_hh, g_bi, g_bh, T, B, in0, H, L, lo, hi,
                                  drop.p, drop.seed, drop.offset, drop.counter_ptr, _stream()), 'halo_lstm_bwd')
    finally:
        if dx_slabs > 1:
            lib().halo_set_lstm_dx_slabs(1)
    return dx, grads


class defer_small_jobs:

    def __enter__(self):
        self.begin()
        return self

    def __exit__(self, *exc):
        self.end()
        return False

    @staticmethod
    def begin():
        check(lib().halo_set_defer_small_jobs(1), 'halo_set_defer_small_jobs')

    @staticmethod
    def end():
        try:
            check(lib().halo_flush_small_jobs(_stream()), 'halo_flush_small_jobs')
        finally:
            lib().halo_set_defer_small_jobs(0)


def lstm_dx_slabs_left():
    return int(lib().halo_lstm_dx_slabs_left())


def log_softmax_fwd(x2d):
    _f32c(x2d, 'logits')
    y = torch.empty_like(x2d)
    check(lib().halo_log_softmax_fwd(ptr(x2d), ptr(y), x2d.shape[0], x2d.shape[1], _stream()), 'halo_log_softmax_fwd')
    return y


def log_softmax_bwd(dy2d, y2d):
    _f32c(dy2d, 'dy'); _f32c(y2d, 'y')
    dx = torch.empty_like(y2d)
    check(lib().halo_log_softmax_bwd(ptr(dy2d), ptr(y2d), ptr(dx), y2d.shape[0], y2d.shape[1], _stream()),
          'halo_log_softmax_bwd')
    return dx


def colsum(x2d, out=None):
    _f32c(x2d, 'x')
# ... 189 lines not shown
    rows, n = values2d.shape
    dev = values2d.device
    vals = torch.empty(rows, k, device=dev, dtype=torch.float32)
    idx = torch.empty(rows, k, device=dev, dtype=torch.int64)
    ws = torch.empty(rows * n * 8, device=dev, dtype=torch.uint8)
    check(lib().halo_topk_f32(ptr(values2d), rows, n, k, ptr(vals), ptr(idx), ptr(ws), _stream()), 'halo_topk_f32')
    return vals, idx


def sumsq_partials(flat, partials=None):
    if partials is None:
        partials = torch.empty(_lib.HALO_SUMSQ_PARTS, device=flat.device, dtype=torch.float32)
    check(lib().halo_sumsq(ptr(flat), flat.numel(), ptr(partials), _stream()), 'halo_sumsq')
    return partials


def _range_arrays(ranges):
    n = len(ranges)
    return n, (C.c_size_t * n)(*[int(r[0]) for r in ranges]), (C.c_size_t * n)(*[int(r[1]) for r in ranges])


def sumsq_ranges(flat, ranges, partials):
    n, b, e = _range_arrays(ranges)
    check(lib().halo_sumsq_ranges(ptr(flat), n, b, e, ptr(partials), _stream()), 'halo_sumsq_ranges')
    return partials


def pack_ranges_bf16(flat, ranges, dst):
    n, b, e = _range_arrays(ranges)
    check(lib().halo_pack_ranges_bf16(ptr(flat), n, b, e, ptr(dst), _stream()), 'halo_pack_ranges_bf16')
    return dst


def expand_ranges_bf16(stage, spans, chunks, world, skip_rank, flat):
    n = len(spans)
    b = (C.c_size_t * n)(*[int(s) for s in spans])
    c = (C.c_size_t * n)(*[int(x) for x in chunks])
    check(lib().halo_expand_ranges_bf16(ptr(stage), n, b, c, int(world), int(skip_rank), ptr(flat), _stream()), 'halo_expand_ranges_bf16')
    return flat


GRAD_SUMSQ_ALL = 31


def collect_grad_sumsq(partials):
    check(lib().halo_set_grad_sumsq(ptr(partials), 0 if partials is None else partials.numel()), 'halo_set_grad_sumsq')


def grad_sumsq_state():
    n, bits = C.c_int(0), C.c_uint(0)
    check(lib().halo_grad_sumsq_state(C.byref(n), C.byref(bits)), 'halo_grad_sumsq_state')
    return int(n.value), int(bits.value)


def clip_coef(partials, count, max_norm, coef, norm, applied_steps=None):
    check(lib().halo_clip_coef_step(ptr(partials), count, float(max_norm), ptr(coef), ptr(norm), ptr(applied_steps), _stream()),
          'halo_clip_coef_step')


def adamw(p, g, m, v, lr, beta1, beta2, eps, weight_decay, step, grad_scale=None):
    _lib.bump_weights_epoch()
    check(lib().halo_adamw(ptr(p), ptr(g), ptr(m), ptr(v), p.numel(), lr, beta1, beta2, eps, weight_decay, step,
                           ptr(grad_scale), _stream()), 'halo_adamw')
    torch.autograd.graph.increment_version(p)


def adamw_ranges(p, g, m, v, ranges, lr, beta1, beta2, eps, step, counter=None):
    _lib.bump_weights_epoch()
    n = len(ranges)
    begin = (C.c_size_t * n)(*[r[0] for r in ranges])
    end = (C.c_size_t * n)(*[r[1] for r in ranges])
    wd = (C.c_float * n)(*[float(r[2]) for r in ranges])
    gs = (C.c_void_p * n)(*[ptr(r[3]) for r in ranges])
    if torch.is_tensor(step):
        lr_dev = lr if torch.is_tensor(lr) else None
        check(lib().halo_adamw_ranges_dev(ptr(p), ptr(g), ptr(m), ptr(v), n, begin, end, wd, gs, 0.0 if lr_dev is not None else lr,
                                          ptr(lr_dev), beta1, beta2, eps, ptr(step), ptr(counter), _stream()), 'halo_adamw_ranges_dev')
    else:
        check(lib().halo_adamw_ranges(ptr(p), ptr(g), ptr(m), ptr(v), n, begin, end, wd, gs, lr, beta1, beta2, eps, step, ptr(counter),
                                      _stream()), 'halo_adamw_ranges')
    torch.autograd.graph.increment_version(p)


class AdamWMulti:

    def __init__(self, params, weight_decays, lr, betas=(0.9, 0.999), eps=1e-8):
        import numpy as np
        self.params = list(params)
        self.wds = [float(w) for w in weight_decays]
        self.param_groups = [{'lr': float(lr), 'params': self.params}]
        self.betas, self.eps = betas, float(eps)
        for p in self.params:
            if p.dtype != torch.float32 or not p.is_contiguous() or not p.is_cuda:
                raise ValueError('AdamWMulti: parameters must be contiguous float32 tensors on the HIP device')
        self.m = [torch.zeros_like(p) for p in self.params]
        self.v = [torch.zeros_like(p) for p in self.params]
        self.t = 0
        dev = self.params[0].device
        chunk, group = lib().halo_adamw_multi_chunk(), lib().halo_adamw_multi_max_tensors()
        assert lib().halo_adamw_multi_tensor_bytes() == 40
        rec = np.dtype([('p', '<u8'), ('m', '<u8'), ('v', '<u8'), ('n', '<u8'), ('decay', '<f4'), ('pad', '<i4')])
        self.groups = []
        for first in range(0, len(self.params), group):
            idx = range(first, min(first + group, len(self.params)))
            table = np.zeros(len(idx), dtype=rec)
            for k, i in enumerate(idx):
                p = self.params[i]
                table[k] = (p.data_ptr(), self.m[i].data_ptr(), self.v[i].data_ptr(), p.numel(), self.wds[i], 0)
            pairs = [(k, c) for k, i in enumerate(idx) for c in range((self.params[i].numel() + chunk - 1) // chunk)]
            self.groups.append((first, len(idx), torch.from_numpy(table.view(np.uint8)).to(dev),
                                torch.tensor(pairs, dtype=torch.int32).view(-1).to(dev), len(pairs)))

    @property
    def lr(self):
        return self.param_groups[0]['lr']

    @lr.setter
    def lr(self, value):
        self.param_groups[0]['lr'] = float(value)

    def step(self, grad_scale=None):
        _lib.bump_weights_epoch()
        self.t += 1
        for first, count, table, chunks, n_chunks in self.groups:
            ptrs = (C.c_void_p * count)()
            for k in range(count):
                p = self.params[first + k]
                g = p.grad
                if g is None or g.dtype != torch.float32 or not g.is_contiguous() or g.device != p.device or g.shape != p.shape:
                    raise ValueError('AdamWMulti.step: every parameter needs a contiguous float32 .grad of its shape on its device')
                ptrs[k] = g.data_ptr()
            check(lib().halo_adamw_multi(ptr(table), ptr(chunks), n_chunks, ptrs, count, self.lr, self.betas[0], self.betas[1], self.eps,
                                         self.t, ptr(grad_scale), _stream()), 'halo_adamw_multi')
        for p in self.params:
            torch.autograd.graph.increment_version(p)


def scale_add_(y, x, alpha, beta, guard=None):
    check(lib().halo_scale_add_guarded(ptr(y), ptr(x), float(alpha), float(beta), y.numel(), ptr(guard), _stream()),
          'halo_scale_add_guarded')
    return y


def cast_f32_to_bf16_(dst_bf16, src_f32):
    check(lib().halo_cast_f32_bf16(ptr(src_f32), ptr(dst_bf16), src_f32.numel(), _stream()), 'halo_cast_f32_bf16')
    return dst_bf16


def cast_bf16_to_f32_(dst_f32, src_bf16, scale=1.0):
    check(lib().halo_cast_bf16_f32(ptr(src_bf16), ptr(dst_f32), float(scale), dst_f32.numel(), _stream()), 'halo_cast_bf16_f32')
    return dst_f32


def counter_inc(counter):
    check(lib().halo_counter_inc(ptr(counter), _stream()), 'halo_counter_inc')


def embed_fwd(ids, wte, wpe, pos0=0):
    ids = _i64c(ids, 'input_ids')
    Bn, T = ids.shape
    C = wte.shape[1]
    x = torch.empty(Bn * T, C, device=wte.device, dtype=torch.float32)
    check(lib().halo_embed_fwd(ptr(ids), ptr(wte), ptr(wpe), ptr(x), Bn * T, T, C, pos0, wte.shape[0], _stream()), 'halo_embed_fwd')
    return x


# ... 444 lines not shown
```

haloop_amd/train.py:

```python
import os
import re
import time

import torch

from . import _lib, _linear, dp, ops
from .ops import Dropout, NO_DROPOUT
from .rnn import lstm_param_list


def decay_groups(encoder, recognizer):
    decay, no_decay = [], []
    for prefix, mod in (('encoder.', encoder), ('recognizer.', recognizer)):
        for name, p in mod.named_parameters():
            is_lstm = name.startswith('lstm.') or name.startswith('rnn.')
            if is_lstm or not name.endswith('bias'):
                decay.append((prefix + name, p))
            else:
                no_decay.append((prefix + name, p))
    return decay, no_decay


def _merge_adjacent(ranges):
    out = []
# ... 61 lines not shown
    def attach_grads(self):
        for n, p, _ in self.slots:
            p.grad = self.grad_views[n]


class LstmCtcTrainer:
    DX_SLABS = int(os.environ.get('HALO_DX_SLABS', '8'))

    def __init__(self, encoder, recognizer, lr=3e-4, betas=(0.9, 0.99), eps=1e-8, weight_decay=0.01,
                 clip_grad_norm=0.1, seed=None, use_graph=True, process_group=None, accumulate=1, grad_dtype='f32',
                 alias_loss=False, fused_head=True, head_one_launch=True, dp_algo='rs_ag', rehearse_dp=False, gather_dtype='f32'):
        self.alias_loss = bool(alias_loss)
        self.fused_head = fused_head
        self.head_one_launch = head_one_launch
        self.encoder, self.recognizer = encoder, recognizer
        self.accumulate = int(accumulate)
        self._micro = 0
        self.betas, self.eps, self.weight_decay, self.clip = betas, eps, weight_decay, clip_grad_norm
        if dp_algo not in ('rs_ag', 'rs_ag_flat', 'allreduce', 'direct'):
            raise ValueError(f"dp_algo must be 'rs_ag', 'direct', 'rs_ag_flat' or 'allreduce', got {dp_algo!r}")
        if gather_dtype not in ('auto', 'f32', 'bf16'):
            raise ValueError(f"gather_dtype must be 'auto', 'f32' or 'bf16', got {gather_dtype!r}")
        self.world = dp.world_size(process_group)
        self.dp_algo = dp_algo if ((self.world > 1 or rehearse_dp) and self.accumulate == 1) else 'allreduce'
        if self.dp_algo in ('rs_ag', 'direct') and grad_dtype == 'bf16':
            self.dp_algo = 'rs_ag_flat'
        self._rehearse_dp = bool(rehearse_dp)
        self.flat = FlatParams(encoder, recognizer, pad_to=4 * self.world if self.dp_algo != 'allreduce' else 4)
        dev = self.flat.params.device
        self._lr_dev = torch.zeros(1, device=dev, dtype=torch.float32)
        self.lr = lr
        self.status = torch.zeros(1, device=dev, dtype=torch.int32)
        _lib.set_status_word(self.status)
        _lib.lend_scratch(device=dev)
        self.device = dev
        self.seed = int(torch.initial_seed() if seed is None else seed) & 0xFFFFFFFFFFFFFFFF
        self.counter = torch.zeros(1, device=dev, dtype=torch.int32)
        self.partials = torch.zeros(_lib.HALO_SUMSQ_PARTS, device=dev, dtype=torch.float32)
        self.partials_p = torch.zeros(4 * _lib.HALO_SUMSQ_PARTS, device=dev, dtype=torch.float32)
        self.coef = torch.ones(2, device=dev, dtype=torch.float32)
        self.grad_norm = torch.zeros(1, device=dev, dtype=torch.float32)
        self.loss = torch.zeros((), device=dev, dtype=torch.float32)
        self.step_count = 0
        self.adam_step = torch.zeros(1, device=dev, dtype=torch.int32)
        self._ticket = torch.zeros(1, device=dev, dtype=torch.int32)
        auto = use_graph == 'auto'
        if auto:
            use_graph = True
        self.use_graph = use_graph
        self._auto = {'n': 0} if (auto and self.world == 1 and not rehearse_dp and self.accumulate == 1) else None
        self.auto_choice = None
        self.eager_forward_backward = os.environ.get('HALO_DP_EAGER_FB', '1') != '0'
        self.pg = process_group
        dp.broadcast_parameters(self.flat.params, process_group)
        self.sharded = None
        self.masters_stale = False
        self._gather_mode = None
        if self.dp_algo in ('rs_ag', 'direct'):
            f = self.flat
            bf16_gather = gather_dtype == 'bf16' or (gather_dtype == 'auto' and _lib.get_math_mode() == 'bf16')
            self._gather_mode = _lib.get_math_mode()
            try:
                if self.dp_algo == 'direct':
                    self.sharded = dp.DirectExchange(f.params, f.grads, f.big_early, f.big_late, f.small_range, process_group,
                                                     gather_bf16=bf16_gather, norm_parts=self.partials.numel())
                else:
                    self.sharded = dp.SpanSharded(f.params, f.grads, f.big_early, f.big_late, f.small_range, process_group,
                                                  always=self._rehearse_dp, gather_bf16=bf16_gather)
            except ValueError as e:
                import logging
                logging.getLogger(__name__).warning('haloop_amd.train: %s; using dp_algo rs_ag_flat', e)
                self.dp_algo = 'rs_ag_flat'
            else:
                self._mid_event = torch.cuda.Event() if dev.type == 'cuda' else None
                if self._mid_event is not None:
                    self._mid_event.record()
        if self.dp_algo == 'rs_ag_flat':
            self.sharded = dp.ShardedUpdate(self.flat.params, self.flat.grads, process_group, always=self._rehearse_dp, wire_dtype=grad_dtype)
        self.avg_early = dp.GradientAverager(self.flat.grads, process_group, span=self.flat.early_range, wire_dtype=grad_dtype)
        self.avg_late = dp.GradientAverager(self.flat.grads, process_group, span=self.flat.late_range, wire_dtype=grad_dtype)
        self._graphs = None
        self._static = None
        self._accum = torch.zeros_like(self.flat.grads) if self.accumulate > 1 else None

    @property
    def lr(self):
        return self._lr

    @lr.setter
    def lr(self, value):
        self._lr = float(value)
        self._lr_dev.fill_(self._lr)

    def check_status(self):
        if int(self.status.item()) != 0:
            raise _lib.HaloError('a persistent LSTM recurrence timed out waiting for its peer workgroups (they were not all resident); '
                                 'no optimizer update has been applied since.  Free the GPU of other work, or select the step-launch '
                                 'chain with haloop_amd._lib.set_lstm_persistent(False), then zero trainer.status and continue.')

    def _dropout(self):
        p = self.encoder.dropout.p if self.encoder.training else 0.0
        return Dropout(p, self.seed, 0, self.counter) if p > 0 else NO_DROPOUT

    def _forward_backward(self, x, il, tg, tl):
        self._backward_rest(self._forward_backward_top(x, il, tg, tl))

    def _forward_backward_top(self, x, il, tg, tl):
        self._defer = not (self.world > 1 and self.dp_algo == 'allreduce')
        if self._defer:
            ops.defer_small_jobs.begin()
        self._norm_count = 0
        self._collect = self._defer and self.world == 1 and self.sharded is None and self.accumulate == 1 and self.encoder.lstm.num_layers == 2
        if self._collect:
            ops.collect_grad_sumsq(self.partials_p)
        try:
            return self._forward_backward_top_body(x, il, tg, tl)
        except BaseException:
            if self._defer:
                self._defer = False
                _lib.lib().halo_set_defer_small_jobs(0)
            if self._collect:
                self._collect = False
                _lib.lib().halo_set_grad_sumsq(None, 0)
            raise

    def _forward_backward_top_body(self, x, il, tg, tl):
        enc, rec, gv = self.encoder, self.recognizer, self.flat.grad_views
        drop = self._dropout()
        B, T, F = x.shape
        L = enc.lstm.num_layers
        lp_list = lstm_param_list(enc.lstm)
        w_ih, w_hh, b_ih, b_hh = lp_list[0::4], lp_list[1::4], lp_list[2::4], lp_list[3::4]
        H, Cc = w_hh[0].shape[1], enc.subsample.weight.shape[0]
        V = rec.classifier.weight.shape[0]
        y_sub, col = ops.subsample_fwd(x, enc.subsample.weight, enc.subsample.bias, drop)
        Tp = y_sub.shape[0]
        feats = torch.empty(B, Tp, H, device=x.device, dtype=torch.float32)
        _, _, _, reserve = ops.lstm_fwd(y_sub, w_ih, w_hh, b_ih, b_hh, y=feats, y_strides=(H, Tp * H), y_relu=True, drop=drop)
        p_cls = rec.dropout.p if rec.training else 0.0
        cdrop = Dropout(p_cls, self.seed, 0, self.counter) if p_cls > 0 else NO_DROPOUT
        grads = {'dw_ih': [gv[f'encoder.lstm.weight_ih_l{k}'] for k in range(L)],
                 'dw_hh': [gv[f'encoder.lstm.weight_hh_l{k}'] for k in range(L)],
                 'db_ih': [gv[f'encoder.lstm.bias_ih_l{k}'] for k in range(L)],
                 'db_hh': [gv[f'encoder.lstm.bias_hh_l{k}'] for k in range(L)]}
        if self.fused_head and ops.ctc_head_supported(Tp, H, V, tg.shape[1]):
            sid = _lib.HALO_STREAM_CLASSIFIER
            if self.head_one_launch and _lib.get_math_mode() != 'f32':
                if getattr(self, '_head_tws', None) is None or self._head_tws_dims != (B, H, V):
                    self._head_tws, self._head_tws_dims = ops.ctc_head_train_workspace(B, H, V, x.device), (B, H, V)
                    self._head_ticket = ops.ctc_head_train_ticket(B, H, x.device)
                dfeats, _, _, _ = ops.ctc_head_train(feats, rec.classifier.weight, rec.classifier.bias, cdrop, sid, il, tg, tl, self.loss,
                                                     self._head_ticket, gv['recognizer.classifier.weight'], gv['recognizer.classifier.bias'],
                                                     workspace=self._head_tws)
                return self._lstm_backward_top(x, y_sub, col, w_ih, w_hh, reserve, grads, drop, dfeats.view(B * Tp, H),
                                               (B, T, F, Cc, H, Tp, L))
            lp, alpha, nll, flen, grad_out, (tg64, tl64) = ops.ctc_head_fwd(feats, rec.classifier.weight, rec.classifier.bias, cdrop, sid,
                                                                           il, tg, tl, self.loss, self._ticket)
            if getattr(self, '_head_ws', None) is None or self._head_ws_dims != (B, H, V):
                self._head_ws, self._head_ws_dims = ops.ctc_head_workspace(B, H, V, x.device), (B, H, V)
            dfeats = ops.ctc_head_bwd(feats, rec.classifier.weight, cdrop, sid, flen, tg64, tl64, lp, alpha, nll, grad_out,
                                      gv['recognizer.classifier.weight'], gv['recognizer.classifier.bias'],
                                      workspace=self._head_ws).view(B * Tp, H)
            return self._lstm_backward_top(x, y_sub, col, w_ih, w_hh, reserve, grads, drop, dfeats, (B, T, F, Cc, H, Tp, L))
        fdrop = ops.dropout_fwd(feats, cdrop, _lib.HALO_STREAM_CLASSIFIER) if p_cls > 0 else feats
        f2d = fdrop.view(B * Tp, H)
        logits = ops.gemm(f2d, rec.classifier.weight, True, True, B * Tp, V, H, bias1=rec.classifier.bias)
        lp = ops.log_softmax_fwd(logits)
        flen, grad_out = ops.ctc_prepare(il, tl)
        nll, alpha, saved = ops.ctc_fwd(lp.view(B, Tp, V), False, tg, flen, tl)
        ops.ctc_mean_loss(nll, tl, self.loss)
        dlp = ops.ctc_bwd(lp.view(B, Tp, V), False, saved, alpha, nll, grad_out)
        dlogits = ops.log_softmax_bwd(dlp.view(B * Tp, V), lp)
        ops.gemm(dlogits, f2d, False, False, V, H, B * Tp, out=gv['recognizer.classifier.weight'])
        ops.colsum(dlogits, out=gv['recognizer.classifier.bias'])
        dfeats = ops.gemm(dlogits, rec.classifier.weight, True, False, B * Tp, H, V, drop=cdrop,
                          stream_id=_lib.HALO_STREAM_CLASSIFIER)
        return self._lstm_backward_top(x, y_sub, col, w_ih, w_hh, reserve, grads, drop, dfeats, (B, T, F, Cc, H, Tp, L))

    def _lstm_backward_top(self, x, y_sub, col, w_ih, w_hh, reserve, grads, drop, dfeats, dims):
        B, T, F, Cc, H, Tp, L = dims
        ws = ops.lstm_bwd_workspace(y_sub, w_hh)
        dy_sub = torch.empty((self.DX_SLABS,) + tuple(y_sub.shape), device=y_sub.device, dtype=torch.float32)
        top = (L - 1 if L > 1 else 0) if (self.world > 1 and self.dp_algo == 'allreduce') else 0
        ops.lstm_bwd(y_sub, w_ih, w_hh, dfeats, (H, Tp * H), True, reserve, grads=grads, drop=drop, layers=(top, L),
                     workspace=ws, dx=dy_sub, dx_slabs=self.DX_SLABS)
        self._dx_slabs = ops.lstm_dx_slabs_left() if top == 0 else 1
        return (y_sub, col, w_ih, w_hh, reserve, grads, drop, ws, dy_sub, top, (B, T, F, Cc, H, Tp, L))

    def _backward_rest(self, st):
        y_sub, col, w_ih, w_hh, reserve, grads, drop, ws, dy_sub, top, (B, T, F, Cc, H, Tp, L) = st
        gv = self.flat.grad_views
        if top > 0:
            if self.world > 1:
                if getattr(self, '_ctx_steps', None) is None:
                    self._ctx_steps = _lib.Context()
                    with self._ctx_steps:
                        _lib.set_lstm_persistent(False)
                with self._ctx_steps:
                    ops.lstm_bwd(y_sub, w_ih, w_hh, None, (H, Tp * H), True, reserve, grads=grads, drop=drop, layers=(0, top),
                                 workspace=ws, dx=dy_sub)
            else:
                ops.lstm_bwd(y_sub, w_ih, w_hh, None, (H, Tp * H), True, reserve, grads=grads, drop=drop, layers=(0, top),
                             workspace=ws, dx=dy_sub)
        try:
            ops.subsample_bwd(dy_sub, y_sub, col, B, T, F, Cc, drop.p, dw=gv['encoder.subsample.weight'],
                              dbias=gv['encoder.subsample.bias'], slabs=self._dx_slabs)
        finally:
            if self._defer:
                self._defer = False
                ops.defer_small_jobs.end()
            if self._collect:
                self._collect = False
                n, bits = ops.grad_sumsq_state()
                ops.collect_grad_sumsq(None)
                self._norm_count = n if bits == ops.GRAD_SUMSQ_ALL else 0

    def _all_reduce(self):
        self.avg_early.average()
        self.avg_late.average()

    def _warm_optimizer_kernels(self):
        dev = self.device
        d = [torch.zeros(8, device=dev, dtype=torch.float32) for _ in range(4)]
        parts = torch.zeros(_lib.HALO_SUMSQ_PARTS, device=dev, dtype=torch.float32)
        coef, norm = torch.ones(2, device=dev, dtype=torch.float32), torch.zeros(1, device=dev, dtype=torch.float32)
        cnt = torch.ones(1, device=dev, dtype=torch.int32)
        ops.sumsq_partials(d[1], parts)
        ops.clip_coef(parts, _lib.HALO_SUMSQ_PARTS, self.clip, coef, norm, applied_steps=cnt)
        ops.adamw_ranges(d[0], d[1], d[2], d[3], [(0, 8, 0.0, coef[0:1])], self.lr, self.betas[0], self.betas[1], self.eps, cnt)

    def _optimizer(self):
        if getattr(self, '_norm_count', 0) > 0 and self.sharded is None:
            self._apply_update(count=self._norm_count)
            return
        self._norm_partials()
        self._apply_update()

    def _own_ranges(self):
        if isinstance(self.sharded, dp.SpanSharded):
            return self.sharded.own_ranges()
        if self.sharded is not None:
            return [self.sharded.span]
        return [(0, self.flat.padded)]

    def _norm_partials(self):
        f = self.flat
        src = self.sharded.norm_ranges() if isinstance(self.sharded, dp.SpanSharded) else self._own_ranges()
        cut = [(max(f.encoder_range[0], lo), min(f.encoder_range[1], hi)) for lo, hi in src]
        cut = _merge_adjacent([(a, b) for a, b in cut if b > a])
        if not cut:
            self.partials.zero_()
        elif len(cut) == 1:
            ops.sumsq_partials(f.grads[cut[0][0]:cut[0][1]], self.partials)
        else:
            ops.sumsq_ranges(f.grads, cut, self.partials)

    def _apply_update(self, count=None):
        f = self.flat
        ops.clip_coef(self.partials_p if count else self.partials, count or _lib.HALO_SUMSQ_PARTS, self.clip, self.coef, self.grad_norm,
                      applied_steps=self.adam_step)
        ranges = [(max(a, lo), min(b, hi), self.weight_decay if decays else 0.0, self.coef[0:1] if clipped else self.coef[1:2])
                  for a, b, decays, clipped in f.ranges for lo, hi in _merge_adjacent(self._own_ranges()) if min(b, hi) > max(a, lo)]
        if ranges:
            ops.adamw_ranges(f.params, f.grads, f.exp_avg, f.exp_avg_sq, ranges, self._lr_dev, self.betas[0], self.betas[1], self.eps,
                             self.adam_step, counter=self.counter)
        else:
            ops.counter_inc(self.counter)

    def _sharded_tail(self):
        sh = self.sharded
        mark = self._dp_mark
        if isinstance(sh, dp.SpanSharded):
            if not self._early_started:
                sh.reduce_scatter('early')
            mark('reduce_scatter_early_tail')
            sh.reduce_scatter('late')
            mark('reduce_scatter_late')
            sh.all_reduce_small()
            mark('all_reduce_small')
        else:
            sh.reduce_scatter()
            mark('reduce_scatter')
        self._norm_partials()
        sh.all_reduce_sum(self.partials)
        mark('norm_partials_and_their_all_reduce')
        self._apply_update()
        mark('clip_and_adamw_on_owned_ranges')
        sh.all_gather()
        mark('all_gather')

    _dp_marks = None

    def _dp_mark(self, name):
        if self._dp_marks is not None:
            ev = torch.cuda.Event(enable_timing=True)
            ev.record()
            self._dp_marks.append((name, ev))

    def profile_dp_components(self, x, il, tg, tl, steps=5):
        if self.sharded is None:
            return None
        was_graph, self.use_graph = self.use_graph, False
        acc = {}
        try:
            for it in range(steps + 1):
                self._dp_marks = []
                start = torch.cuda.Event(enable_timing=True)
                start.record()
                self._early_started = False
                self.masters_stale = bool(getattr(self.sharded, 'gather_bf16', False))
                handle = self._forward_backward_overlapped(x, il, tg, tl)
                self._dp_mark('forward_backward')
                if handle is not None:
                    self.sharded.wait(handle)
                    self._early_started = True
                self._dp_mark('wait_early_reduce_scatter')
                self._sharded_tail()
                torch.cuda.synchronize()
                if it > 0:
                    prev = start
                    for name, ev in self._dp_marks:
                        acc[name] = acc.get(name, 0.0) + 1e3 * prev.elapsed_time(ev) / steps
                        prev = ev
                    acc['step_total'] = acc.get('step_total', 0.0) + 1e3 * start.elapsed_time(prev) / steps
        finally:
            self._dp_marks = None
            self.use_graph = was_graph
        return {k: round(v, 1) for k, v in acc.items()}

    def gather_master_weights(self):
        if isinstance(self.sharded, dp.SpanSharded) and self.sharded.gather_bf16:
            self.sharded.gather_masters()
            _lib.bump_weights_epoch()
        self.masters_stale = False

    def state_dict(self):
        if self.masters_stale:
            self.gather_master_weights()
        return {'encoder': self.encoder.state_dict(), 'recognizer': self.recognizer.state_dict()}

    def step(self, x, input_lengths, targets, target_lengths):
        if self._auto is not None:
            loss = self._auto_step(x, input_lengths, targets, target_lengths)
        else:
            loss = self._step(x, input_lengths, targets, target_lengths)
        return loss if self.alias_loss else loss.clone()

    _AUTO = (8, 28, 33, 53)

    def _auto_step(self, x, il, tg, tl):
        a, (w0, g1, w1, e1) = self._auto, self._AUTO
        a['n'] += 1
        n = a['n']
        if n == w0 + 1 or n == w1 + 1:
            torch.cuda.synchronize()
            a['t0'] = time.perf_counter()
        self.use_graph = n <= g1
        loss = self._step(x, il, tg, tl)
        if n == g1 or n == e1:
            torch.cuda.synchronize()
            a['graph' if n == g1 else 'eager'] = time.perf_counter() - a['t0']
        if n == e1:
            self.use_graph = not (a['eager'] / (e1 - w1) < 0.99 * a['graph'] / (g1 - w0))
            self.auto_choice = {'graph_replay_ms': 1e3 * a['graph'] / (g1 - w0), 'eager_launches_ms': 1e3 * a['eager'] / (e1 - w1),
                                'use_graph': self.use_graph}
            self._auto = None
        return loss

    def _step(self, x, input_lengths, targets, target_lengths):
        if _lib._status_tensor is not self.status:
            _lib.set_status_word(self.status)
        if self.accumulate > 1:
            return self._accumulating_step(x, input_lengths, targets, target_lengths)
        self.step_count += 1
        if self.sharded is not None:
            if self._gather_mode is not None and getattr(self.sharded, 'gather_bf16', False) and _lib.get_math_mode() != self._gather_mode:
                self.gather_master_weights()
                self.sharded.gather_bf16 = False
                self._tail_graph, self._tail_calls = None, 0
            return self._sharded_step(x, input_lengths, targets, target_lengths)
        if not self.use_graph:
            st = self._forward_backward_top(x, input_lengths, targets, target_lengths)
            w1 = self.avg_early.start()
            self._backward_rest(st)
            w2 = self.avg_late.start()
            self.avg_early.finish(w1)
            self.avg_late.finish(w2)
            self._optimizer()
            return self.loss
        return self._graph_step(x, input_lengths, targets, target_lengths)

    def _forward_backward_overlapped(self, x, il, tg, tl):
        sh = self.sharded
        ev = self._mid_event if (isinstance(sh, dp.SpanSharded) and (sh._native or getattr(sh, 'side_ok', False)) and 'early' in sh.spans) else None
        if ev is None:
            self._forward_backward(x, il, tg, tl)
            return None
        _lib.set_lstm_bwd_mid_event(ev)
        try:
            st = self._forward_backward_top(x, il, tg, tl)
            recorded = _lib.lib().halo_lstm_bwd_mid_event_recorded() == 1
        finally:
            _lib.set_lstm_bwd_mid_event(None)
        handle = sh.reduce_scatter('early', after=ev) if recorded else None
        self._backward_rest(st)
        return handle

    def _sharded_step(self, x, il, tg, tl):
        handle = None
        self._early_started = False
        self.masters_stale = bool(getattr(self.sharded, 'gather_bf16', False))
        if not self.use_graph or self.eager_forward_backward:
            handle = self._forward_backward_overlapped(x, il, tg, tl)
        else:
            self._replay_forward_backward(x, il, tg, tl)
        if handle is not None:
            self.sharded.wait(handle)
            self._early_started = True
        if not self.use_graph:
            self._sharded_tail()
            return self.loss
        self._tail_calls = getattr(self, '_tail_calls', 0) + 1
        want_capture = os.environ.get('HALO_DP_CAPTURE', '1' if self.world == 1 else '0') != '0'
        if self._tail_calls == 2 and self.sharded._native and want_capture:
            try:
                torch.cuda.synchronize()
                g = torch.cuda.CUDAGraph()
                with torch.cuda.graph(g, capture_error_mode='thread_local'):
                    self._sharded_tail()
                self._tail_graph, self._tail_graph_early = g, self._early_started
            except Exception as e:
                import logging
                logging.getLogger(__name__).warning('haloop_amd.train: capturing the collectives failed (%s: %s); they run eagerly',
                                                    type(e).__name__, e)
                torch.cuda.synchronize()
                self._tail_graph = None
        if getattr(self, '_tail_graph', None) is not None and self._tail_graph_early == self._early_started:
            _lib.bump_weights_epoch()
            self._tail_graph.replay()
        else:
            self._sharded_tail()
        return self.loss

    def _accumulating_step(self, x, il, tg, tl):
        if self.use_graph:
            self._replay_forward_backward(x, il, tg, tl)
        else:
            self._forward_backward(x, il, tg, tl)
        self._micro += 1
        first, last = self._micro == 1, self._micro == self.accumulate
        ops.scale_add_(self._accum, self.flat.grads, 0.0 if first else 1.0, 1.0 / self.accumulate, guard=self.loss)
        if not last:
            ops.counter_inc(self.counter)
            return self.loss
        self._micro = 0
        self.flat.grads.copy_(self._accum)
        self._all_reduce()
        self.step_count += 1
        self._optimizer()
        return self.loss

    def _replay_forward_backward(self, x, il, tg, tl):
        if self._graphs is None or len(self._graphs) != 1 or self._static[0].shape != x.shape or self._static[2].shape != tg.shape:
            self._static = tuple(t.contiguous().clone() for t in (x, il.to(torch.int64), tg.to(torch.int64), tl.to(torch.int64)))
            sx, sil, stg, stl = self._static
            side = torch.cuda.Stream()
            side.wait_stream(torch.cuda.current_stream())
            with torch.cuda.stream(side):
                self._forward_backward(sx, sil, stg, stl)
            torch.cuda.current_stream().wait_stream(side)
            g = torch.cuda.CUDAGraph()
            with torch.cuda.graph(g):
                self._forward_backward(sx, sil, stg, stl)
            self._graphs = (g,)
        for dst, src in zip(self._static, (x, il, tg, tl)):
            if src.data_ptr() != dst.data_ptr():
                dst.copy_(src)
        _lib.bump_weights_epoch()
        self._graphs[0].replay()

    def _graph_step(self, x, il, tg, tl):
        if self._graphs is None or self._static[0].shape != x.shape or self._static[2].shape != tg.shape:
            self._static = tuple(t.contiguous().clone() for t in (x, il.to(torch.int64), tg.to(torch.int64), tl.to(torch.int64)))
            sx, sil, stg, stl = self._static
            side = torch.cuda.Stream()
            side.wait_stream(torch.cuda.current_stream())
            with torch.cuda.stream(side):
                self._forward_backward(sx, sil, stg, stl)
                self._warm_optimizer_kernels()
            torch.cuda.current_stream().wait_stream(side)
            if self.world == 1:
                g = torch.cuda.CUDAGraph()
                with torch.cuda.graph(g):
                    self._forward_backward(sx, sil, stg, stl)
                    self._optimizer()
                self._graphs = (g,)
            else:
                g1, g2, g3 = torch.cuda.CUDAGraph(), torch.cuda.CUDAGraph(), torch.cuda.CUDAGraph()
                torch.cuda.synchronize()
                mode = dict(capture_error_mode='thread_local')
                with torch.cuda.graph(g1, **mode):
                    state = self._forward_backward_top(sx, sil, stg, stl)
                with torch.cuda.graph(g2, pool=g1.pool(), **mode):
                    self._backward_rest(state)
                with torch.cuda.graph(g3, pool=g1.pool(), **mode):
                    self._optimizer()
                self._graphs = (g1, g2, g3)
                self._keep = state
        sx, sil, stg, stl = self._static
        for dst, src in ((sx, x), (sil, il), (stg, tg), (stl, tl)):
            if src.data_ptr() != dst.data_ptr():
                dst.copy_(src)
        if len(self._graphs) == 1:
            _lib.bump_weights_epoch()
            self._graphs[0].replay()
        else:
            _lib.bump_weights_epoch()
            self._graphs[0].replay()
            w1 = self.avg_early.start()
            _lib.bump_weights_epoch()
            self._graphs[1].replay()
            w2 = self.avg_late.start()
            self.avg_early.finish(w1)
            self.avg_late.finish(w2)
            _lib.bump_weights_epoch()
            self._graphs[2].replay()
        return self.loss

    def static_inputs(self):
        return self._static


class GraphedTrainStep:

    def __init__(self, forward, params, dropout_streams=()):
        self.forward = forward
        self.params = [p for p in params if p.requires_grad]
        self.streams = list(dropout_streams)
        dev = self.params[0].device
        self.counter = torch.zeros(1, device=dev, dtype=torch.int32)
        for s in self.streams:
            s.counter = self.counter
        self._graph = self._static = self._loss = None

    def _run(self, inputs):
        with _linear.graphed_run():
            loss = self.forward(*inputs)
            with torch.autograd.set_multithreading_enabled(False):
                loss.backward()
        if self.streams:
            ops.counter_inc(self.counter)
        return loss

    def step(self, *inputs):
        shapes = tuple((tuple(t.shape), t.dtype) for t in inputs)
        if self._graph is None or self._shapes != shapes:
            self._shapes = shapes
            self._static = tuple(t.detach().clone() for t in inputs)
            for p in self.params:
                p.grad = None
            side = torch.cuda.Stream()
            side.wait_stream(torch.cuda.current_stream())
            with torch.cuda.stream(side):
                for _ in range(2):
                    for p in self.params:
                        p.grad = None
                    self._run(self._static)
            torch.cuda.current_stream().wait_stream(side)
            for p in self.params:
                p.grad = None
            graph = torch.cuda.CUDAGraph()
            with torch.cuda.graph(graph):
                self._loss = self._run(self._static)
            self._graph = graph
        for dst, src in zip(self._static, inputs):
            dst.copy_(src)
        _lib.bump_weights_epoch()
        self._graph.replay()
        return self._loss.detach().clone()
# ... 1 lines not shown
```

include/halo.h:

```cpp
#ifndef HALO_H
#define HALO_H

#include <stddef.h>
#include <stdint.h>

#ifdef __cplusplus
extern "C" {
#endif

#define HALO_ABI_VERSION 19

#define HALO_OK 0
#define HALO_EINVAL (-22)
#define HALO_ENOTSUP (-95)
#define HALO_ELAUNCH (-5)

typedef void *halo_stream_t;

int halo_abi_version(void);
int halo_debug_read(const void *src, size_t bytes, int pattern, size_t row_bytes, float *sink, void *stream);
const char *halo_strerror(int code);
int halo_device_info(int device, char *arch, int arch_len, int *cu_count);

#define HALO_MATH_F32 0
#define HALO_MATH_BF16X3 1
#define HALO_MATH_BF16 2
int halo_set_math_mode(int mode);
int halo_get_math_mode(void);

int halo_set_lstm_fusion(int on);

int halo_set_scratch(void *device_ptr, size_t bytes);

#define HALO_STREAM_SUBSAMPLE 1u
#define HALO_STREAM_CLASSIFIER 2u
#define HALO_STREAM_LSTM_LAYER0 16u

int halo_dropout_fwd(const float *x, float *y, size_t n, float p, uint64_t seed, uint32_t stream_id,
                     uint32_t offset, const uint32_t *offset_dev, halo_stream_t stream);
int halo_counter_inc(uint32_t *counter, halo_stream_t stream);

#define HALO_GEMM_RELU 1
#define HALO_GEMM_GELU 2
#define HALO_GEMM_ACCUM 4
#define HALO_GEMM_GELU_ERF 8
int halo_gemm_f32(int a_kcontig, int b_kcontig, int M, int N, int K, const float *A, int lda,
                  const float *B, int ldb, float *C, int ldc, const float *bias1, const float *bias2,
                  int flags, float p_drop, uint64_t seed, uint32_t stream_id, uint32_t offset,
                  const uint32_t *offset_dev, halo_stream_t stream);

size_t halo_split_image_bytes(int rows, int k);
int halo_split_image(const float *src, int rows, int k, int ld, int src_transposed, void *image,
                     halo_stream_t stream);
int halo_layernorm_image(const float *x, const float *weight, const float *bias, float *y, void *image, int rows, int C,
                         float eps, halo_stream_t stream);
int halo_layernorm_bf16(const float *x, const float *weight, const float *bias, float *y, void *y_bf16, void *image, int rows, int C,
                        float eps, halo_stream_t stream);
int halo_cast_bf16(const float *x, void *y, size_t n, halo_stream_t stream);
int halo_gelu_bf16(const float *a, void *y_bf16, size_t n, int exact, halo_stream_t stream);
int halo_gelu_bwd_bf16(const float *dy, const float *a, void *da_bf16, size_t n, int exact, halo_stream_t stream);
int halo_gelu_b16(const void *a_bf16, void *y_bf16, size_t n, int exact, halo_stream_t stream);
int halo_gelu_bwd_b16(const void *dy_bf16, const void *a_bf16, void *da_bf16, size_t n, int exact, halo_stream_t stream);
#define HALO_PAIR_COPY 0
#define HALO_PAIR_GELU_TANH 1
#define HALO_PAIR_GELU_ERF 2
#define HALO_PAIR_GELU_TANH_BWD 3
#define HALO_PAIR_GELU_ERF_BWD 4
int halo_image_pair(const float *src, const float *src2, int rows, int cols, long ld, long ld2, int op, void *image_rows,
                    void *image_cols, halo_stream_t stream);
int halo_cross_entropy_bwd_images(const float *logits, const int64_t *targets, const float *lse, const float *grad,
                                  long grad_stride, int rows, int V, long ld, long ignore_index, void *image_rows,
                                  void *image_cols, halo_stream_t stream);
int halo_image_pairs(int n, const float *const *src, const int *rows, const int *cols, const long *ld, void *const *image_rows,
                     void *const *image_cols, halo_stream_t stream);
int halo_gemm_split(const void *a_image, const void *b_image, int M, int N, int K, float *C, int ldc,
                    const float *bias1, const float *bias2, int flags, float p_drop, uint64_t seed,
                    uint32_t stream_id, uint32_t offset, const uint32_t *offset_dev, halo_stream_t stream);

int halo_gemm_split_residual(const void *a_image, const void *b_image, int M, int N, int K, float *C, int ldc, const float *residual,
                             int ldr, const float *bias1, const float *bias2, int flags, float p_drop, uint64_t seed,
                             uint32_t stream_id, uint32_t offset, const uint32_t *offset_dev, halo_stream_t stream);

int halo_gemm_tn_bf16(const void *a, long lda, const void *b, long ldb, int M, int N, int K, float *C, int ldc, int flags,
                      halo_stream_t stream);
int halo_gemm_tn_bf16_group(int n, const void *const *a, const long *lda, const void *const *b, const long *ldb, const int *M, const int *N, int K,
                            float *const *C, const int *ldc, int flags, halo_stream_t stream);

int halo_gemm_tn_rows_supported(int n, const int *M, const int *N, int K);
int halo_gemm_tn_rows_preferred(int n, const int *M, const int *N, int K);
int halo_gemm_tn_rows_group(int n, const void *const *a, const long *lda, const void *const *b, const long *ldb, const int *M, const int *N, int K,
                            float *const *C, const long *ldc, halo_stream_t stream);

int halo_gemm_split_io(const void *a_image, const void *a_hi, const void *a_lo, long lda, const void *b_image, int M, int N, int K, float *C,
                       int ldc, void *out_hi, void *out_lo, long ldo, const float *residual, int ldr, const float *bias1,
                       const float *bias2, int flags, halo_stream_t stream);

int halo_attention_fwd_b16(const void *q, long q_row_stride, long q_batch_stride, const void *k, const void *v, long kv_row_stride,
                           long kv_batch_stride, float *y, long y_row_stride, long y_batch_stride, void *y_bf16, long yb_row_stride,
                           long yb_batch_stride, float *lse, int N, int heads, int head_dim, int Tq, int Tk, int causal, halo_stream_t stream);
int halo_attention_bwd_b16(const void *q, long q_row_stride, long q_batch_stride, const void *k, const void *v, long kv_row_stride,
                           long kv_batch_stride, const void *y_bf16, const void *dy_bf16, long y_row_stride, long y_batch_stride, const float *lse,
                           float *delta, void *dq_bf16, void *dk_bf16, void *dv_bf16, long d_row_stride, long d_batch_stride, int N, int heads,
                           int head_dim, int Tq, int Tk, int causal, halo_stream_t stream);

int halo_gemm_rows_supported(int M, int N, int K);
int halo_gemm_rows(const void *a_image, const void *a_bf16, long lda, const void *b_image, int M, int N, int K, float *C, long ldc,
                   const float *residual, long ldr, void *out_bf16, long ldo, halo_stream_t stream);
int halo_gemm_rows_gelu(const void *a_image, const void *a_bf16, long lda, const void *b_image, int M, int N, int K, void *out_bf16,
                        void *pre_bf16, long ldo, int exact, halo_stream_t stream);
size_t halo_gemm_rows_ce_workspace_bytes(int M, int N);
int halo_gemm_rows_ce(const void *a_image, const void *a_bf16, long lda, const void *b_image, int M, int N, int K, const int64_t *targets,
                      long ignore_index, void *workspace, float *loss, float *lse, void *logits_bf16, long ldo, halo_stream_t stream);
int halo_cross_entropy_bwd_bf16(void *logits_bf16, const int64_t *targets, const float *lse, const float *grad, long grad_stride, int rows,
                                int V, long ld, long ignore_index, halo_stream_t stream);

size_t halo_gemm_split_ce_workspace_bytes(int M, int N);
int halo_gemm_split_ce(const void *a_image, const void *b_image, int M, int N, int K, float *logits, int ldc, const float *bias,
                       const int64_t *targets, long ignore_index, void *workspace, float *loss, float *lse, halo_stream_t stream);

size_t halo_subsample_col_bytes(int B, int T, int F, int ks, int stride, int pad);
int halo_subsample_fwd(const float *x, const float *w, const float *bias, float *y, float *col, int B,
                       int T, int F, int C, int ks, int stride, int pad, float p_drop, uint64_t seed,
                       uint32_t offset, const uint32_t *offset_dev, halo_stream_t stream);
int halo_subsample_bwd(const float *dy, const float *y, const float *col, float *dpre, float *dw,
                       float *dbias, int B, int T, int F, int C, int ks, int stride, int pad, float p_drop,
                       halo_stream_t stream);
int halo_subsample_bwd_slabs(float *dy, int slabs, const float *y, const float *col, float *dpre, float *dw,
                             float *dbias, int B, int T, int F, int C, int ks, int stride, int pad, float p_drop,
                             halo_stream_t stream);

size_t halo_lstm_reserve_bytes(int T, int B, int in0, int H, int L);
size_t halo_lstm_bwd_workspace_bytes(int T, int B, int in0, int H, int L);
int halo_lstm_fwd(const float *x, const float *const *w_ih, const float *const *w_hh,
                  const float *const *b_ih, const float *const *b_hh, const float *h0, const float *c0,
                  float *y, long y_stride_t, long y_stride_b, int y_relu, float *hn, float *cn,
                  float *reserve, int T, int B, int in0, int H, int L, float p_drop, uint64_t seed,
                  uint32_t offset, const uint32_t *offset_dev, halo_stream_t stream);
int halo_lstm_bwd(const float *x, const float *const *w_ih, const float *const *w_hh, const float *dy,
                  long y_stride_t, long y_stride_b, int y_relu, const float *dhn, const float *dcn,
                  float *reserve, float *workspace, float *dx, float *const *dw_ih, float *const *dw_hh,
                  float *const *db_ih, float *const *db_hh, int T, int B, int in0, int H, int L,
                  int layer_begin, int layer_end, float p_drop, uint64_t seed, uint32_t offset,
                  const uint32_t *offset_dev, halo_stream_t stream);

typedef struct halo_ctx halo_ctx;
halo_ctx *halo_ctx_create(void);
void halo_ctx_destroy(halo_ctx *ctx);
int halo_ctx_use(halo_ctx *ctx);
int halo_set_status_word(uint32_t *device_word);
int halo_debug_mute_workgroup(int block);
int halo_debug_mfma_clock(unsigned long long *ticks, float *sink, int blocks, int iters, int shape, unsigned seed, halo_stream_t stream);

int halo_set_lstm_persistent(int on);
int halo_set_lstm_persistent_images(int on);
int halo_lstm_persistent_eligible(int B, int H);
int halo_set_lstm_persistent2(int on);
int halo_set_lstm_interleave(int on);
int halo_set_gemm256(int on);
int halo_set_lstm_bwd_mid_event(void *event);
int halo_lstm_bwd_mid_event_recorded(void);
int halo_set_lstm_weights_stamp(uint64_t stamp);
int halo_set_lstm_expect_backward(int on);
int halo_set_lstm_dx_slabs(int n);
int halo_lstm_dx_slabs_left(void);
int halo_set_defer_small_jobs(int on);
int halo_flush_small_jobs(halo_stream_t stream);
int halo_set_grad_sumsq(float *partials, int capacity);
int halo_grad_sumsq_state(int *count, unsigned *covered);
int halo_lstm_persistent2_eligible(int T, int B, int H, int L);
size_t halo_lstm_status_offset(int backward, int T, int B, int in0, int H, int L);

int halo_lstm_persist_stamps(void *device_buffer);

int halo_lstm_chain_events(void *ev_begin, void *ev_end);
int halo_lstm_chain_info(int backward, int *launches, char *kernel, int kernel_len);

int halo_log_softmax_fwd(const float *x, float *y, int rows, int cols, halo_stream_t stream);
int halo_log_softmax_bwd(const float *dy, const float *y, float *dx, int rows, int cols,
                         halo_stream_t stream);
int halo_colsum(const float *x, int rows, int cols, int ld, float *out, halo_stream_t stream);

#define HALO_CTC_FULL_LATTICE 1
#define HALO_CTC_FINITE_MIN 2
#define HALO_CTC_NO_LEAD_BLANK_LOOP 4
#define HALO_CTC_WRAP_SKIP 8
int halo_ctc_fwd(const float *lp, long stride_t, long stride_n, int T, int N, int C,
                 const int64_t *targets, long tg_stride, int S, const int64_t *input_lengths,
                 const int64_t *target_lengths, int flags, float *alpha, float *nll,
                 halo_stream_t stream);
int halo_ctc_bwd(const float *lp, long stride_t, long stride_n, int T, int N, int C,
                 const int64_t *targets, long tg_stride, int S, const int64_t *input_lengths,
                 const int64_t *target_lengths, const float *alpha, const float *nll,
                 const float *grad_out, float *beta, float *grad, long gstride_t, long gstride_n,
                 halo_stream_t stream);

int halo_ctc_prepare(const int64_t *input_lengths, const int64_t *target_lengths, int n, int ks, int stride,
                     int pad, int64_t *feature_lengths, float *grad_out, halo_stream_t stream);
int halo_ctc_mean_loss(const float *nll, const int64_t *target_lengths, int n, float *loss,
                       halo_stream_t stream);

int halo_ctc_head_greedy(const float *features, const float *weight, const float *bias, float *lp, int64_t *alignments, float *scores,
                         int64_t *hyp, int64_t *hyp_len, int B, int T, int H, int V, halo_stream_t stream);
int halo_ctc_head_supported(int T, int H, int V, int S);
size_t halo_ctc_head_workspace_bytes(int B, int H, int V);
int halo_ctc_head_fwd(const float *features, const float *weight, const float *bias, float p_drop, uint64_t seed,
                      uint32_t stream_id, uint32_t offset, const uint32_t *offset_dev, const int64_t *input_lengths, int ks,
                      int stride, int pad, const int64_t *targets, long tg_stride, int S, const int64_t *target_lengths,
                      float *lp, float *alpha, float *nll, int64_t *feature_lengths, float *grad_out, float *loss,
                      uint32_t *ticket, int B, int T, int H, int V, halo_stream_t stream);
int halo_ctc_head_bwd(const float *features, const float *weight, float p_drop, uint64_t seed, uint32_t stream_id,
                      uint32_t offset, const uint32_t *offset_dev, const int64_t *feature_lengths, const int64_t *targets,
                      long tg_stride, int S, const int64_t *target_lengths, const float *lp, const float *alpha,
                      const float *nll, const float *grad_out, float *dfeatures, float *dweight, float *dbias,
                      void *workspace, int B, int T, int H, int V, halo_stream_t stream);

size_t halo_ctc_head_train_workspace_bytes(int B, int H, int V);
size_t halo_ctc_head_train_ticket_words(int B, int H);
int halo_ctc_head_train(const float *features, const float *weight, const float *bias, float p_drop, uint64_t seed,
                        uint32_t stream_id, uint32_t offset, const uint32_t *offset_dev, const int64_t *input_lengths, int ks,
                        int stride, int pad, const int64_t *targets, long tg_stride, int S, const int64_t *target_lengths,
                        float *lp, float *nll, int64_t *feature_lengths, float *loss, uint32_t *ticket, float *dfeatures,
                        float *dweight, float *dbias, void *workspace, int B, int T, int H, int V, halo_stream_t stream);

int halo_ctc_greedy(const float *lp, int N, int T, int C, int64_t *alignments, float *scores,
                    int64_t *hyp, int64_t *hyp_len, halo_stream_t stream);

int halo_fbank_frames(const float *wav, long n_samples, int frame_len, int shift, int padded, float preemphasis, int remove_dc,
                      const float *window, float *frames, int n_frames, halo_stream_t stream);
int halo_fbank_power(const float *spectrum, int n_frames, int bins, float *power, int ld, halo_stream_t stream);
int halo_fbank_log(float *x, long n, float eps, halo_stream_t stream);
int halo_fbank_spectrum_mel(const float *frames, int n_frames, int padded, const double *twiddle, const double *banks, int num_bins,
                            float eps, float *out, halo_stream_t stream);

size_t halo_star_ctc_workspace_bytes(int T, int N, int S);
int halo_star_ctc_fwd(const float *log_probs, long stride_t, long stride_n, int T, int N, int C, const int64_t *targets, int S,
                      const int64_t *emission_lengths, const int64_t *target_lengths, float star_penalty, void *workspace,
                      float *losses, halo_stream_t stream);
int halo_star_ctc_bwd(const float *log_probs, long stride_t, long stride_n, int T, int N, int C, const int64_t *targets, int S,
                      const int64_t *emission_lengths, const int64_t *target_lengths, float star_penalty,
                      const void *workspace, const float *losses, const float *grad_losses, float *grad_log_probs,
                      halo_stream_t stream);
size_t halo_transducer_workspace_bytes(int N, int T, int U1);
int halo_transducer_fwd(const float *joint, int N, int T, int U1, int K, const int64_t *targets, const int *joint_lengths,
                        const int *target_lengths, void *workspace, float *losses, halo_stream_t stream);
int halo_transducer_bwd(const float *joint, int N, int T, int U1, int K, const int64_t *targets, const int *joint_lengths,
// ... 73 lines not shown
                       uint64_t seed, uint32_t stream_id, uint32_t offset, const uint32_t *offset_dev,
                       halo_stream_t stream);
int halo_attention_masked(const float *q, const float *k, const float *v, const unsigned char *mask, long mask_stride_n, long mask_stride_h,
                          long mask_stride_t, float *y, float *entropy, int N, int heads, int T, int S, int head_dim, halo_stream_t stream);
int halo_attention_fwd_bf16(const float *q, long q_row_stride, long q_batch_stride, const float *k, const float *v, long kv_row_stride,
                            long kv_batch_stride, float *y, long y_row_stride, long y_batch_stride, void *y_bf16, long ybf_row_stride,
                            long ybf_batch_stride, float *lse, int N, int heads, int head_dim, int Tq, int Tk, int causal,
                            const int *key_lengths, float p_drop, uint64_t seed, uint32_t stream_id, uint32_t offset,
                            const uint32_t *offset_dev, halo_stream_t stream);
int halo_attention_bwd_bf16(const float *q, long q_row_stride, long q_batch_stride, const float *k, const float *v, long kv_row_stride,
                            long kv_batch_stride, const float *y, const float *dy, long y_row_stride, long y_batch_stride, const float *lse,
                            float *delta, void *dq_bf16, void *dk_bf16, void *dv_bf16, long d_row_stride, long d_batch_stride, int N,
                            int heads, int head_dim, int Tq, int Tk, int causal, const int *key_lengths, float p_drop, uint64_t seed,
                            uint32_t stream_id, uint32_t offset, const uint32_t *offset_dev, halo_stream_t stream);
size_t halo_layernorm_bwd_workspace_bytes(int rows, int C);
int halo_layernorm_bwd(const float *dy, const float *x, const float *weight, const float *dres, float *dx,
                       float *dweight, float *dbias, void *workspace, int rows, int C, float eps,
                       halo_stream_t stream);
int halo_layernorm_bwd_bf16(const float *dy, const float *x, const float *weight, const float *dres, float *dx, void *dx_bf16,
                            float *dweight, float *dbias, void *workspace, int rows, int C, float eps, halo_stream_t stream);
int halo_layernorm_bwd_b16(const void *dy_bf16, const float *x, const float *weight, const float *dres, float *dx, void *dx_bf16, float *dweight,
                           float *dbias, void *workspace, int rows, int C, float eps, halo_stream_t stream);
int halo_gelu_fwd(const float *a, float *y, size_t n, int exact, halo_stream_t stream);
int halo_gelu_bwd(const float *dy, const float *a, float *da, size_t n, int exact, halo_stream_t stream);
int halo_cross_entropy_fwd_lse(const float *logits, const int64_t *targets, float *loss, float *lse, int rows, int V,
                               long ld, long ignore_index, halo_stream_t stream);
int halo_cross_entropy_bwd(float *logits, const int64_t *targets, const float *lse, const float *grad,
                           long grad_stride, int rows, int V, long ld, long ignore_index, halo_stream_t stream);
int halo_embed_bwd(const int64_t *ids, const float *dx, float *dwte, float *dwpe, int B, int T, int C, int pos0,
                   int vocab, int accumulate_wpe, halo_stream_t stream);
int halo_add_rows_bcast(float *x, const float *p, int rows, int T, int C, halo_stream_t stream);

int halo_im2col_cl(const float *x, float *col, int N, int T, int Cin, int ks, int stride, int pad,
                   halo_stream_t stream);
int halo_col2im_cl(const float *dcol, float *dx, int N, int T, int Cin, int ks, int stride, int pad,
                   halo_stream_t stream);
int halo_dwconv1d_cl(const float *x, const float *weight, const float *bias, float *y, int N, int T, int C, int ks,
                     int stride, int pad, halo_stream_t stream);
size_t halo_dwconv1d_cl_bwd_workspace_bytes(int C, int ks);
int halo_dwconv1d_cl_bwd(const float *dy, const float *x, const float *weight, float *dx, float *dweight,
                         float *dbias, void *workspace, int N, int T, int C, int ks, int stride, int pad,
                         halo_stream_t stream);

int halo_tape_batch(const void *data, int elem_bytes, long n_tokens, int batch_size, int bptt_len, long part_index,
                    int rows, long pad_value, void *out, halo_stream_t stream);
int halo_lm_batch_u16(const uint16_t *data, long n_tokens, const int64_t *offsets, int B, int T, int objective_cond,
                      int64_t *x, int64_t *y, halo_stream_t stream);

#define HALO_SUMSQ_PARTS 1024
int halo_scale_add(float *y, const float *x, float alpha, float beta, size_t n, halo_stream_t stream);
int halo_scale_add_guarded(float *y, const float *x, float alpha, float beta, size_t n, const float *guard,
                           halo_stream_t stream);
int halo_cast_f32_bf16(const float *x, void *y_bf16, size_t n, halo_stream_t stream);
int halo_cast_bf16_f32(const void *x_bf16, float *y, float scale, size_t n, halo_stream_t stream);
int halo_sumsq(const float *x, size_t n, float *partials, halo_stream_t stream);
int halo_dx_alloc(size_t bytes, void **ptr, void *handle64);
int halo_dx_open(const void *handle64, void **ptr);
int halo_dx_close(void *ptr);
int halo_dx_free(void *ptr);
int halo_dx_push(const void *src, size_t piece_bytes, size_t piece_stride_bytes, int same, void *const *peer_bases, size_t dst_offset, int world,
                 int rank, halo_stream_t stream);
int halo_dx_signal(void *const *peer_bases, size_t flag_offset, int world, int rank, uint32_t epoch, halo_stream_t stream);
int halo_dx_wait(const void *own_flags, int world, int rank, uint32_t epoch, halo_stream_t stream);
int halo_dx_reduce(float *own, const float *inbox, size_t elems, int world, int rank, float scale, halo_stream_t stream);

int halo_sumsq_ranges(const float *x, int n, const size_t *begin, const size_t *end, float *partials, halo_stream_t stream);
int halo_pack_ranges_bf16(const float *src, int n, const size_t *begin, const size_t *end, void *dst, halo_stream_t stream);
int halo_expand_ranges_bf16(const void *stage, int n, const size_t *begin, const size_t *chunk, int world, int skip_rank, float *dst,
                            halo_stream_t stream);
int halo_clip_coef(const float *partials, int count, float max_norm, float *coef, float *norm_out,
                   halo_stream_t stream);
int halo_clip_coef_step(const float *partials, int count, float max_norm, float *coef, float *norm_out,
                        uint32_t *applied_steps, halo_stream_t stream);
int halo_adamw(float *p, const float *g, float *m, float *v, size_t n, float lr, float beta1, float beta2,
               float eps, float weight_decay, int step, const float *grad_scale, halo_stream_t stream);
int halo_adamw_ranges(float *p, const float *g, float *m, float *v, int n_ranges, const size_t *begin, const size_t *end,
                      const float *weight_decay, const float *const *grad_scale, float lr, float beta1, float beta2,
                      float eps, int step, uint32_t *counter, halo_stream_t stream);

int halo_adamw_ranges_dev(float *p, const float *g, float *m, float *v, int n_ranges, const size_t *begin, const size_t *end,
                          const float *weight_decay, const float *const *grad_scale, float lr, const float *lr_dev, float beta1,
                          float beta2, float eps, const uint32_t *step_dev, uint32_t *counter, halo_stream_t stream);

size_t halo_adamw_multi_tensor_bytes(void);
unsigned halo_adamw_multi_chunk(void);
int halo_adamw_multi_max_tensors(void);
int halo_adamw_multi(const void *tensor_table, const void *chunk_table, int n_chunks, const float *const *grads, int n_tensors,
                     float lr, float beta1, float beta2, float eps, int step, const float *grad_scale, halo_stream_t stream);

#ifdef __cplusplus
}
#endif
#endif
```

Measured before the change: 159,900 utterances/s.

## Emit bf16 LSTM weight tile images from AdamW to skip forward repacking

Adds a fused AdamW kernel that, for the three recurrent weight matrices used by the persistent two-layer LSTM path, updates the weights and writes their bf16 forward and transposed tile images straight into a persistent reserve buffer. The next forward pass checks that the images are current (same reserve, weights and dims) and skips the pack-pair tiling blocks. This removes a separate read and repack of about 12M weight elements per step. In exchange it adds version tracking, a persistent reserve tied to the shapes, and a transposing epilogue in the optimizer, which could cost more than it saves.

Measured after the change: 162,200 utterances/s, median of 6. 1.01x the previous value.

```diff
diff --git a/haloop_amd/_lib.py b/haloop_amd/_lib.py
--- a/haloop_amd/_lib.py
+++ b/haloop_amd/_lib.py
@@ -4,7 +4,8 @@
 _HERE = os.path.dirname(os.path.abspath(__file__))
 LIB_PATH = os.path.join(_HERE, 'csrc', 'libhalo.so')
 
-HALO_ABI_VERSION = 19
+HALO_ABI_VERSION = 20
+HALO_EINVAL = -22
 HALO_GEMM_RELU = 1
 HALO_GEMM_GELU = 2
 HALO_GEMM_ACCUM = 4
@@ -90,6 +91,10 @@
     'halo_set_lstm_bwd_mid_event': (_i, [_vp]),
     'halo_lstm_bwd_mid_event_recorded': (_i, []),
     'halo_set_lstm_expect_backward': (_i, [_i]),
+    'halo_lstm_persist2_image_ptrs': (_i, [_vp, _i, _i, _i, _i, _i, _vp, _vp]),
+    'halo_lstm_persist2_pack_images': (_i, [_vp, _vp, _vp, _vp, _i, _i, _i, _i, _i, _vp]),
+    'halo_set_lstm_images_current': (_i, [_vp, _vp, _vp, _vp, _i, _i, _i, _i, _i]),
+    'halo_lstm_persist2_last_tile_blocks': (_i, []),
     'halo_set_lstm_dx_slabs': (_i, [_i]),
     'halo_set_defer_small_jobs': (_i, [_i]),
     'halo_set_grad_sumsq': (_i, [_vp, _i]),
@@ -189,6 +194,7 @@
     'halo_scale_add_guarded': (_i, [_vp, _vp, _f, _f, _sz, _vp, _vp]),
     'halo_clip_coef_step': (_i, [_vp, _i, _f, _vp, _vp, _vp, _vp]),
     'halo_adamw_ranges_dev': (_i, [_vp, _vp, _vp, _vp, _i, _vp, _vp, _vp, _vp, _f, _vp, _f, _f, _f, _vp, _vp, _vp]),
+    'halo_adamw_ranges_emit_dev': (_i, [_vp, _vp, _vp, _vp, _i, _vp, _vp, _vp, _vp, _f, _vp, _f, _f, _f, _vp, _vp, _i, _vp, _i, _vp, _vp, _vp]),
     'halo_ctx_create': (_vp, []),
     'halo_ctx_destroy': (None, [_vp]),
     'halo_ctx_use': (_i, [_vp]),
diff --git a/haloop_amd/csrc/halo_internal.h b/haloop_amd/csrc/halo_internal.h
--- a/haloop_amd/csrc/halo_internal.h
+++ b/haloop_amd/csrc/halo_internal.h
@@ -53,6 +53,9 @@
     uint64_t lstm_weights_stamp = 0, packF_stamp = 0;
     const float *packF_reserve = nullptr, *packF_w[3] = {nullptr, nullptr, nullptr};
     int packF_dims[5] = {0, 0, 0, 0, 0};
+    const float *cur_reserve = nullptr, *cur_w[3] = {nullptr, nullptr, nullptr};
+    int cur_dims[5] = {0, 0, 0, 0, 0};
+    int last_tile_blocks = -1;
     int mute_block = -1;
 };
 HaloCtx &halo_ctx_cur();
diff --git a/haloop_amd/csrc/lstm.hip b/haloop_amd/csrc/lstm.hip
--- a/haloop_amd/csrc/lstm.hip
+++ b/haloop_amd/csrc/lstm.hip
@@ -1221,7 +1221,8 @@
 int lstm_fwd_persist2(const float *in, int in_dim, int lo, const float *const *w_ih, const float *const *w_hh, const float *const *b_ih,
                       const float *const *b_hh, const float *h0, const float *c0, float *y, long y_stride_t, long y_stride_b,
                       int y_relu, float *hn, float *cn, float *reserve, float *extra, char *img_in, char *img_w, int T, int B,
-                      int in0, int H, int L, float p_drop, uint64_t seed, uint32_t offset, const uint32_t *offset_dev, hipStream_t st) {
+                      int in0, int H, int L, float p_drop, uint64_t seed, uint32_t offset, const uint32_t *offset_dev, bool images_current,
+                      hipStream_t st) {
     const int hi = lo + 1;
     const size_t BH = (size_t)B * H;
     const LayerBufs l0 = layer_bufs(reserve, lo, T, B, H), l1 = layer_bufs(reserve, hi, T, B, H);
@@ -1266,7 +1267,8 @@
         PackPairArgs pp;
         for (int m = 0; m < 3; ++m) { pp.w[m] = pa.w[m]; pp.fwd[m] = (char *)pa.wdst[m]; pp.tr[m] = (char *)(wT + (size_t)m * 4 * H * H); }
         pp.H = H;
-        pp.tile_blocks = 3 * (4 * H / 32) * (H / 32) / 4;
+        pp.tile_blocks = images_current ? 0 : 3 * (4 * H / 32) * (H / 32) / 4;
+        ctx.last_tile_blocks = pp.tile_blocks;
         pp.rest = pa; pp.rest.w_units = 0;
         pp.rest.zero2 = reserve_bwd_flags(reserve, T, B, in0, H, L); pp.rest.zero2_units = (long)(PERSIST_FLAG_BYTES / 16);
         pp.zbase[0] = pp.zbase[1] = nullptr; pp.zstride = 0; pp.zunits = 0; pp.zcount = 0;
@@ -1436,6 +1438,55 @@
     halo_ctx_cur().lstm_expect_backward = on ? 1 : 0;
     return HALO_OK;
 }
+
+namespace {
+int persist2_image_ptrs(float *reserve, int T, int B, int in0, int H, int L, char **fwd, char **tr) {
+    if (!reserve || T <= 0 || B <= 0 || in0 <= 0 || H <= 0 || L < 2 || H % 32 != 0) return HALO_EINVAL;
+    if (fused_ok(H, L) || !use_x3(H) || !halo_lstm_persist2_ok(T, B, H, L)) return HALO_EINVAL;
+    const int kin = in0 > H ? in0 : H;
+    char *img_in = (char *)(reserve + (size_t)4 * H * H + (size_t)L * layer_floats(T, B, H));
+    char *img_w = img_in + halo_tiled_image_bytes(T * B, kin);
+    float *extra = (float *)(img_w + halo_tiled_image_bytes(4 * H, kin));
+    float *wp1 = fused_wpk(extra, L - 1, H);
+    float *wT = (float *)((char *)reserve + reserve_flags_offset(T, B, in0, H, L) + PERSIST_FLAG_BYTES);
+    fwd[0] = (char *)reserve; fwd[1] = (char *)wp1; fwd[2] = (char *)(wp1 + (size_t)4 * H * H);
+    for (int m = 0; m < 3; ++m) tr[m] = (char *)(wT + (size_t)m * 4 * H * H);
+    return HALO_OK;
+}
+}
+
+int halo_lstm_persist2_image_ptrs(float *reserve, int T, int B, int in0, int H, int L, void **fwd_images, void **tr_images) {
+    HALO_CHECK_ARG(fwd_images && tr_images);
+    char *fwd[3], *tr[3];
+    const int rc = persist2_image_ptrs(reserve, T, B, in0, H, L, fwd, tr);
+    if (rc != HALO_OK) return rc;
+    for (int m = 0; m < 3; ++m) { fwd_images[m] = fwd[m]; tr_images[m] = tr[m]; }
+    return HALO_OK;
+}
+
+int halo_lstm_persist2_pack_images(const float *w_hh_lo, const float *w_hh_hi, const float *w_ih_hi, float *reserve, int T, int B, int in0,
+                                   int H, int L, halo_stream_t stream) {
+    HALO_CHECK_ARG(w_hh_lo && w_hh_hi && w_ih_hi);
+    PackPairArgs pp = {};
+    const int rc = persist2_image_ptrs(reserve, T, B, in0, H, L, pp.fwd, pp.tr);
+    if (rc != HALO_OK) return rc;
+    pp.w[0] = w_hh_lo; pp.w[1] = w_hh_hi; pp.w[2] = w_ih_hi;
+    pp.H = H;
+    pp.tile_blocks = 3 * (4 * H / 32) * (H / 32) / 4;
+    hipLaunchKernelGGL(persist2_pack_pair_kernel, dim3((unsigned)pp.tile_blocks), dim3(256), 0, (hipStream_t)stream, pp);
+    return halo_launch_status();
+}
+
+int halo_set_lstm_images_current(const float *reserve, const float *w_hh_lo, const float *w_hh_hi, const float *w_ih_hi, int T, int B, int in0,
+                                 int H, int L) {
+    HaloCtx &ctx = halo_ctx_cur();
+    ctx.cur_reserve = reserve;
+    ctx.cur_w[0] = w_hh_lo; ctx.cur_w[1] = w_hh_hi; ctx.cur_w[2] = w_ih_hi;
+    ctx.cur_dims[0] = T; ctx.cur_dims[1] = B; ctx.cur_dims[2] = in0; ctx.cur_dims[3] = H; ctx.cur_dims[4] = L;
+    return HALO_OK;
+}
+
+int halo_lstm_persist2_last_tile_blocks(void) { return halo_ctx_cur().last_tile_blocks; }
 int halo_lstm_persistent2_eligible(int T, int B, int H, int L) {       return !fused_ok(H, L) && use_x3(H) && halo_lstm_persist2_ok(T, B, H, L) ? 1 : 0; }
 
 size_t halo_lstm_status_offset(int backward, int T, int B, int in0, int H, int L) {
@@ -1461,6 +1512,16 @@
     const size_t BH = (size_t)B * H, PH = bt16(B) * H;
     halo_ctx_cur().packT_reserve = nullptr;
     halo_ctx_cur().emitT_reserve = nullptr;
+    bool images_current = false;
+    {
+        HaloCtx &ctx = halo_ctx_cur();
+        const int dims[5] = {T, B, in0, H, L};
+        images_current = ctx.cur_reserve && ctx.cur_reserve == reserve && L >= 2 && ctx.lstm_expect_backward && H % 32 == 0 &&
+                         !memcmp(ctx.cur_dims, dims, sizeof(dims)) && w_hh[L - 2] && ctx.cur_w[0] == w_hh[L - 2] &&
+                         ctx.cur_w[1] == w_hh[L - 1] && ctx.cur_w[2] == w_ih[L - 1];
+        ctx.cur_reserve = nullptr;
+        ctx.last_tile_blocks = -1;
+    }
     float *wp = reserve;
     const bool x3 = use_x3(H);
     const int kin = in0 > H ? in0 : H;
@@ -1489,7 +1550,7 @@
         if (pair && l == n_single) {
             float *extra = (float *)(img_w + halo_tiled_image_bytes(4 * H, kin));
             return lstm_fwd_persist2(in, in_dim, l, w_ih, w_hh, b_ih, b_hh, h0, c0, y, y_stride_t, y_stride_b, y_relu, hn, cn, reserve, extra,
-                                     img_in, img_w, T, B, in0, H, L, p_drop, seed, offset, offset_dev, st);
+                                     img_in, img_w, T, B, in0, H, L, p_drop, seed, offset, offset_dev, images_current, st);
         }
         if (halo_math_mode() != HALO_MATH_F32 && in_dim >= 64) {
             const HaloPrepJob jobs[2] = {{0, in, T * B, in_dim, in_dim, img_in, nullptr}, {0, w_ih[l], 4 * H, in_dim, in_dim, img_w, nullptr}};
diff --git a/haloop_amd/csrc/optim.hip b/haloop_amd/csrc/optim.hip
--- a/haloop_amd/csrc/optim.hip
+++ b/haloop_amd/csrc/optim.hip
@@ -204,6 +204,128 @@
         }
     }
     if (a.counter && blockIdx.x == 0 && threadIdx.x == 0) *a.counter += 1u;
+}
+
+constexpr int ADAM_MAX_MATS = 3;
+struct AdamEmitMats {
+    size_t off[ADAM_MAX_MATS];
+    char *fwd[ADAM_MAX_MATS], *tr[ADAM_MAX_MATS];
+    float decay_mul[ADAM_MAX_MATS], weight_decay[ADAM_MAX_MATS];
+    const float *grad_scale[ADAM_MAX_MATS];
+    int H, n;
+    unsigned panel_blocks;
+};
+
+template <bool NT, bool PNT>
+__global__ __launch_bounds__(256) void adamw_emit_kernel(const AdamRangesArgs a, const AdamEmitMats mt) {
+    typedef __bf16 bf16x8 __attribute__((ext_vector_type(8)));
+    __shared__ __attribute__((aligned(16))) float tile[32][132];
+    float step_size = a.step_size, bc2_sqrt = a.bc2_sqrt;
+    const float lr = a.lr_dev ? *a.lr_dev : a.lr;
+    if (a.step_dev) {
+        const double t = (double)max(*a.step_dev, 1u);
+        step_size = (float)((double)lr / (1.0 - pow((double)a.beta1, t)));
+        bc2_sqrt = (float)sqrt(1.0 - pow((double)a.beta2, t));
+    }
+    if (blockIdx.x < mt.panel_blocks) {
+        const int wave = threadIdx.x >> 6, lane = threadIdx.x & 63;
+        const int H = mt.H, nkb = H / 32, nkb4 = 4 * H / 32;
+        const int panels_c = H / 128, panels_per = (4 * H / 32) * panels_c;
+        const int m = (int)(blockIdx.x / panels_per), pp = (int)(blockIdx.x % panels_per);
+        const int R0 = (pp / panels_c) * 32, Cp = (pp % panels_c) * 128;
+        const float gs = mt.grad_scale[m] ? *mt.grad_scale[m] : 1.0f;
+        const bool skip = gs != gs;
+        const float decay_mul = a.lr_dev ? (float)(1.0 - (double)lr * (double)mt.weight_decay[m]) : mt.decay_mul[m];
+        const int lrow = wave * 8 + (lane >> 5), lcol = (lane & 31) * 4;
+        const size_t e0 = mt.off[m] + (size_t)(R0 + lrow) * H + Cp + lcol;
+        f32x4 p[4];
+        if (skip) {
+#pragma unroll
+            for (int q = 0; q < 4; ++q) p[q] = *reinterpret_cast<const f32x4 *>(a.p + e0 + (size_t)q * 2 * H);
+        } else {
+            f32x4 gr[4], mo[4], vo[4];
+#pragma unroll
+            for (int q = 0; q < 4; ++q) {
+                const size_t e = e0 + (size_t)q * 2 * H;
+                p[q] = *reinterpret_cast<const f32x4 *>(a.p + e);
+                if (NT) {
+                    gr[q] = __builtin_nontemporal_load(reinterpret_cast<const f32x4 *>(a.g + e));
+                    mo[q] = __builtin_nontemporal_load(reinterpret_cast<const f32x4 *>(a.m + e));
+                    vo[q] = __builtin_nontemporal_load(reinterpret_cast<const f32x4 *>(a.v + e));
+                } else {
+                    gr[q] = *reinterpret_cast<const f32x4 *>(a.g + e);
+                    mo[q] = *reinterpret_cast<const f32x4 *>(a.m + e);
+                    vo[q] = *reinterpret_cast<const f32x4 *>(a.v + e);
+                }
+            }
+#pragma unroll
+            for (int q = 0; q < 4; ++q) {
+                const size_t e = e0 + (size_t)q * 2 * H;
+#pragma unroll
+                for (int c = 0; c < 4; ++c) {
+                    const float ge = mt.grad_scale[m] ? gr[q][c] * gs : gr[q][c];
+                    float pe = p[q][c], me = mo[q][c], ve = vo[q][c];
+                    adam_update(pe, me, ve, ge, decay_mul, a.beta1_w, a.beta2, a.beta2_w, step_size, bc2_sqrt, a.eps);
+                    p[q][c] = pe; mo[q][c] = me; vo[q][c] = ve;
+                }
+                if (PNT) __builtin_nontemporal_store(p[q], reinterpret_cast<f32x4 *>(a.p + e));
+                else *reinterpret_cast<f32x4 *>(a.p + e) = p[q];
+                if (NT) {
+                    __builtin_nontemporal_store(mo[q], reinterpret_cast<f32x4 *>(a.m + e));
+                    __builtin_nontemporal_store(vo[q], reinterpret_cast<f32x4 *>(a.v + e));
+                } else {
+                    *reinterpret_cast<f32x4 *>(a.m + e) = mo[q];
+                    *reinterpret_cast<f32x4 *>(a.v + e) = vo[q];
+                }
+            }
+        }
+#pragma unroll
+        for (int q = 0; q < 4; ++q) *reinterpret_cast<f32x4 *>(&tile[lrow + q * 2][lcol]) = p[q];
+        __syncthreads();
+        const int C0 = Cp + wave * 32, tc = wave * 32;
+        const int i = lane & 15, kg = lane >> 4;
+        const int g = R0 / H, jt = (R0 % H) / 16;
+#pragma unroll
+        for (int half = 0; half < 2; ++half) {
+            const f32x4 v0 = *reinterpret_cast<const f32x4 *>(&tile[half * 16 + i][tc + kg * 8]);
+            const f32x4 v1 = *reinterpret_cast<const f32x4 *>(&tile[half * 16 + i][tc + kg * 8 + 4]);
+            bf16x8 hi;
+#pragma unroll
+            for (int e = 0; e < 4; ++e) { hi[e] = (__bf16)v0[e]; hi[4 + e] = (__bf16)v1[e]; }
+            *reinterpret_cast<bf16x8 *>(mt.fwd[m] + (((long)(jt + half) * 4 + g) * nkb + C0 / 32) * 2048 + lane * 16) = hi;
+        }
+#pragma unroll
+        for (int c = 0; c < 2; ++c) {
+            bf16x8 hi;
+#pragma unroll
+            for (int e = 0; e < 8; ++e) hi[e] = (__bf16)tile[kg * 8 + e][tc + c * 16 + i];
+            *reinterpret_cast<bf16x8 *>(mt.tr[m] + ((long)(C0 / 16 + c) * nkb4 + R0 / 32) * 2048 + lane * 16) = hi;
+        }
+        return;
+    }
+    f32x4 *p4 = reinterpret_cast<f32x4 *>(a.p), *m4 = reinterpret_cast<f32x4 *>(a.m), *v4 = reinterpret_cast<f32x4 *>(a.v);
+    const f32x4 *g4 = reinterpret_cast<const f32x4 *>(a.g);
+    const unsigned fb = blockIdx.x - mt.panel_blocks, nfb = gridDim.x - mt.panel_blocks;
+    for (int r = 0; r < a.n_ranges; ++r) {
+        const float gs = a.grad_scale[r] ? *a.grad_scale[r] : 1.0f;
+        if (gs != gs) continue;
+        const float decay_mul = a.lr_dev ? (float)(1.0 - (double)lr * (double)a.weight_decay[r]) : a.decay_mul[r];
+        for (size_t i = a.begin4[r] + fb * (size_t)256 + threadIdx.x; i < a.end4[r]; i += (size_t)nfb * 256) {
+            f32x4 p = p4[i], m = NT ? __builtin_nontemporal_load(m4 + i) : m4[i], v = NT ? __builtin_nontemporal_load(v4 + i) : v4[i];
+            const f32x4 g = NT ? __builtin_nontemporal_load(g4 + i) : g4[i];
+#pragma unroll
+            for (int e = 0; e < 4; ++e) {
+                const float ge = a.grad_scale[r] ? g[e] * gs : g[e];
+                float pe = p[e], me = m[e], ve = v[e];
+                adam_update(pe, me, ve, ge, decay_mul, a.beta1_w, a.beta2, a.beta2_w, step_size, bc2_sqrt, a.eps);
+                p[e] = pe; m[e] = me; v[e] = ve;
+            }
+            p4[i] = p;
+            if (NT) { __builtin_nontemporal_store(m, m4 + i); __builtin_nontemporal_store(v, v4 + i); }
+            else { m4[i] = m; v4[i] = v; }
+        }
+    }
+    if (a.counter && fb == 0 && threadIdx.x == 0) *a.counter += 1u;
 }
 
 struct AdamTensor {
@@ -484,6 +606,74 @@
     return halo_launch_status();
 }
 
+int halo_adamw_ranges_emit_dev(float *p, const float *g, float *m, float *v, int n_ranges, const size_t *begin, const size_t *end,
+                               const float *weight_decay, const float *const *grad_scale, float lr, const float *lr_dev, float beta1,
+                               float beta2, float eps, const uint32_t *step_dev, uint32_t *counter, int n_mats, const size_t *mat_offset,
+                               int H, void *const *fwd_images, void *const *tr_images, halo_stream_t stream) {
+    HALO_CHECK_ARG(p && g && m && v && begin && end && weight_decay && grad_scale && n_ranges > 0 && n_ranges <= ADAM_MAX_RANGES && step_dev);
+    HALO_CHECK_ARG(((uintptr_t)p % 16 == 0) && ((uintptr_t)g % 16 == 0) && ((uintptr_t)m % 16 == 0) && ((uintptr_t)v % 16 == 0));
+    HALO_CHECK_ARG(n_mats >= 1 && n_mats <= ADAM_MAX_MATS && mat_offset && fwd_images && tr_images && H >= 128 && H % 128 == 0);
+    const size_t mat_len = (size_t)4 * H * H;
+    AdamEmitMats mt;
+    mt.H = H; mt.n = n_mats;
+    mt.panel_blocks = (unsigned)n_mats * (unsigned)(4 * H / 32) * (unsigned)(H / 128);
+    for (int k = 0; k < n_mats; ++k) {
+        HALO_CHECK_ARG(mat_offset[k] % 4 == 0 && fwd_images[k] && tr_images[k] && ((uintptr_t)fwd_images[k] % 16 == 0) &&
+                       ((uintptr_t)tr_images[k] % 16 == 0));
+        HALO_CHECK_ARG(k == 0 || mat_offset[k] >= mat_offset[k - 1] + mat_len);
+        mt.off[k] = mat_offset[k]; mt.fwd[k] = (char *)fwd_images[k]; mt.tr[k] = (char *)tr_images[k];
+    }
+    AdamRangesArgs a;
+    a.p = p; a.g = g; a.m = m; a.v = v; a.n_ranges = 0; a.counter = counter;
+    a.step_dev = step_dev; a.lr_dev = lr_dev; a.lr = lr; a.beta1 = beta1;
+    size_t biggest = 0;
+    int placed = 0;
+    auto piece = [&](size_t lo, size_t hi, int r) {
+        if (hi <= lo) return true;
+        if (a.n_ranges == ADAM_MAX_RANGES) return false;
+        const int k = a.n_ranges++;
+        a.begin4[k] = lo / 4; a.end4[k] = hi / 4;
+        a.decay_mul[k] = (float)(1.0 - (double)lr * (double)weight_decay[r]);
+        a.weight_decay[k] = weight_decay[r];
+        a.grad_scale[k] = grad_scale[r];
+        if (a.end4[k] - a.begin4[k] > biggest) biggest = a.end4[k] - a.begin4[k];
+        return true;
+    };
+    for (int r = 0; r < n_ranges; ++r) {
+        HALO_CHECK_ARG(begin[r] % 4 == 0 && end[r] % 4 == 0 && begin[r] <= end[r]);
+        size_t cur = begin[r];
+        for (int k = 0; k < n_mats; ++k) {
+            if (mt.off[k] < cur || mt.off[k] + mat_len > end[r]) continue;
+            HALO_CHECK_ARG(piece(cur, mt.off[k], r));
+            cur = mt.off[k] + mat_len;
+            mt.decay_mul[k] = (float)(1.0 - (double)lr * (double)weight_decay[r]);
+            mt.weight_decay[k] = weight_decay[r];
+            mt.grad_scale[k] = grad_scale[r];
+            ++placed;
+        }
+        HALO_CHECK_ARG(piece(cur, end[r], r));
+    }
+    HALO_CHECK_ARG(placed == n_mats);
+    for (int k = 0; k < n_mats; ++k)
+        for (int r = 0; r < a.n_ranges; ++r) HALO_CHECK_ARG(a.end4[r] * 4 <= mt.off[k] || a.begin4[r] * 4 >= mt.off[k] + mat_len);
+    a.beta1_w = (float)(1.0 - (double)beta1);
+    a.beta2 = beta2;
+    a.beta2_w = (float)(1.0 - (double)beta2);
+    a.step_size = 0.f; a.bc2_sqrt = 0.f;
+    a.eps = eps;
+    size_t flat = (biggest + 255) / 256;
+    if (flat > 1024) flat = 1024;
+    if (flat < 1) flat = 1;
+    static int nt = -1, pnt = -1;
+    if (nt < 0) { const char *e = getenv("HALO_ADAMW_NT"); nt = (e && e[0] == '0') ? 0 : 1; }
+    if (pnt < 0) { const char *e = getenv("HALO_ADAMW_P_NT"); pnt = (e && e[0] == '1') ? 1 : 0; }
+    const dim3 grid(mt.panel_blocks + (unsigned)flat);
+    if (nt && pnt) hipLaunchKernelGGL((adamw_emit_kernel<true, true>), grid, dim3(256), 0, (hipStream_t)stream, a, mt);
+    else if (nt) hipLaunchKernelGGL((adamw_emit_kernel<true, false>), grid, dim3(256), 0, (hipStream_t)stream, a, mt);
+    else hipLaunchKernelGGL((adamw_emit_kernel<false, false>), grid, dim3(256), 0, (hipStream_t)stream, a, mt);
+    return halo_launch_status();
+}
+
 int halo_adamw_ranges(float *p, const float *g, float *m, float *v, int n_ranges, const size_t *begin, const size_t *end,
                       const float *weight_decay, const float *const *grad_scale, float lr, float beta1, float beta2, float eps, int step,
                       uint32_t *counter, halo_stream_t stream) {
diff --git a/haloop_amd/ops.py b/haloop_amd/ops.py
--- a/haloop_amd/ops.py
+++ b/haloop_amd/ops.py
@@ -401,6 +401,25 @@
     return torch.empty((lib().halo_lstm_reserve_bytes(T, B, in0, H, L) + 3) // 4, device=device, dtype=torch.float32)
 
 
+def lstm_persist2_image_ptrs(reserve, T, B, in0, H, L):
+    fwd, tr = (C.c_void_p * 3)(), (C.c_void_p * 3)()
+    rc = lib().halo_lstm_persist2_image_ptrs(ptr(reserve), T, B, in0, H, L, fwd, tr)
+    if rc == _lib.HALO_EINVAL:
+        return None
+    check(rc, 'halo_lstm_persist2_image_ptrs')
+    return [int(a) for a in fwd], [int(a) for a in tr]
+
+
+def lstm_persist2_pack_images(w_hh_lo, w_hh_hi, w_ih_hi, reserve, T, B, in0, H, L):
+    check(lib().halo_lstm_persist2_pack_images(ptr(w_hh_lo), ptr(w_hh_hi), ptr(w_ih_hi), ptr(reserve), T, B, in0, H, L, _stream()),
+          'halo_lstm_persist2_pack_images')
+
+
+def set_lstm_images_current(reserve, w_hh_lo, w_hh_hi, w_ih_hi, T, B, in0, H, L):
+    check(lib().halo_set_lstm_images_current(ptr(reserve), ptr(w_hh_lo), ptr(w_hh_hi), ptr(w_ih_hi), T, B, in0, H, L),
+          'halo_set_lstm_images_current')
+
+
 def lstm_bwd_workspace(x_tm, w_hh):
     T, B, in0 = x_tm.shape
     return torch.empty((lib().halo_lstm_bwd_workspace_bytes(T, B, in0, w_hh[0].shape[1], len(w_hh)) + 3) // 4,
@@ -756,6 +775,21 @@
     torch.autograd.graph.increment_version(p)
 
 
+def adamw_ranges_emit(p, g, m, v, ranges, lr, beta1, beta2, eps, step, counter, mat_offsets, H, fwd_images, tr_images):
+    _lib.bump_weights_epoch()
+    n, k = len(ranges), len(mat_offsets)
+    begin = (C.c_size_t * n)(*[r[0] for r in ranges])
+    end = (C.c_size_t * n)(*[r[1] for r in ranges])
+    wd = (C.c_float * n)(*[float(r[2]) for r in ranges])
+    gs = (C.c_void_p * n)(*[ptr(r[3]) for r in ranges])
+    lr_dev = lr if torch.is_tensor(lr) else None
+    check(lib().halo_adamw_ranges_emit_dev(ptr(p), ptr(g), ptr(m), ptr(v), n, begin, end, wd, gs, 0.0 if lr_dev is not None else lr,
+                                           ptr(lr_dev), beta1, beta2, eps, ptr(step), ptr(counter), k, (C.c_size_t * k)(*mat_offsets), H,
+                                           (C.c_void_p * k)(*fwd_images), (C.c_void_p * k)(*tr_images), _stream()),
+          'halo_adamw_ranges_emit_dev')
+    torch.autograd.graph.increment_version(p)
+
+
 class AdamWMulti:
 
     def __init__(self, params, weight_decays, lr, betas=(0.9, 0.999), eps=1e-8):
diff --git a/haloop_amd/train.py b/haloop_amd/train.py
--- a/haloop_amd/train.py
+++ b/haloop_amd/train.py
@@ -167,6 +167,9 @@
         self._graphs = None
         self._static = None
         self._accum = torch.zeros_like(self.flat.grads) if self.accumulate > 1 else None
+        self._emit = None
+        self._emit_on = False
+        self._graph_emit = False
 
     @property
     def lr(self):
@@ -221,7 +224,13 @@
         y_sub, col = ops.subsample_fwd(x, enc.subsample.weight, enc.subsample.bias, drop)
         Tp = y_sub.shape[0]
         feats = torch.empty(B, Tp, H, device=x.device, dtype=torch.float32)
-        _, _, _, reserve = ops.lstm_fwd(y_sub, w_ih, w_hh, b_ih, b_hh, y=feats, y_strides=(H, Tp * H), y_relu=True, drop=drop)
+        emit = self._emit if self._emit_on else None
+        if emit is not None and emit['key'] != (Tp, B, Cc, H, L):
+            emit, self._emit_on = None, False
+        if emit is not None:
+            ops.set_lstm_images_current(emit['reserve'], w_hh[L - 2], w_hh[L - 1], w_ih[L - 1], Tp, B, Cc, H, L)
+        _, _, _, reserve = ops.lstm_fwd(y_sub, w_ih, w_hh, b_ih, b_hh, y=feats, y_strides=(H, Tp * H), y_relu=True, drop=drop,
+                                        reserve=None if emit is None else emit['reserve'])
         p_cls = rec.dropout.p if rec.training else 0.0
         cdrop = Dropout(p_cls, self.seed, 0, self.counter) if p_cls > 0 else NO_DROPOUT
         grads = {'dw_ih': [gv[f'encoder.lstm.weight_ih_l{k}'] for k in range(L)],
@@ -313,6 +322,11 @@
         ops.sumsq_partials(d[1], parts)
         ops.clip_coef(parts, _lib.HALO_SUMSQ_PARTS, self.clip, coef, norm, applied_steps=cnt)
         ops.adamw_ranges(d[0], d[1], d[2], d[3], [(0, 8, 0.0, coef[0:1])], self.lr, self.betas[0], self.betas[1], self.eps, cnt)
+        if self._emit_on:
+            n = 4 * 128 * 128
+            e = [torch.zeros(n, device=dev, dtype=torch.float32) for _ in range(6)]
+            ops.adamw_ranges_emit(e[0], e[1], e[2], e[3], [(0, n, 0.0, coef[0:1])], self.lr, self.betas[0], self.betas[1], self.eps, cnt, None,
+                                  [0], 128, [e[4].data_ptr()], [e[5].data_ptr()])
 
     def _optimizer(self):
         if getattr(self, '_norm_count', 0) > 0 and self.sharded is None:
@@ -346,11 +360,74 @@
                       applied_steps=self.adam_step)
         ranges = [(max(a, lo), min(b, hi), self.weight_decay if decays else 0.0, self.coef[0:1] if clipped else self.coef[1:2])
                   for a, b, decays, clipped in f.ranges for lo, hi in _merge_adjacent(self._own_ranges()) if min(b, hi) > max(a, lo)]
-        if ranges:
+        if ranges and self._emit_on:
+            mats = sorted(zip(self._emit['offsets'], self._emit['fwd'], self._emit['tr']))
+            ops.adamw_ranges_emit(f.params, f.grads, f.exp_avg, f.exp_avg_sq, ranges, self._lr_dev, self.betas[0], self.betas[1], self.eps,
+                                  self.adam_step, self.counter, [o for o, _, _ in mats], self._emit['key'][3], [a for _, a, _ in mats],
+                                  [a for _, _, a in mats])
+        elif ranges:
             ops.adamw_ranges(f.params, f.grads, f.exp_avg, f.exp_avg_sq, ranges, self._lr_dev, self.betas[0], self.betas[1], self.eps,
                              self.adam_step, counter=self.counter)
         else:
             ops.counter_inc(self.counter)
+
+    def _emit_key(self, x):
+        if os.environ.get('HALO_ADAMW_EMIT', '1') == '0' or self.sharded is not None or self.world != 1 or self.accumulate != 1:
+            return None
+        lstm = getattr(self.encoder, 'lstm', None)
+        if lstm is None or lstm.num_layers < 2 or _lib.get_math_mode() != 'bf16' or x.dim() != 3:
+            return None
+        H = lstm.weight_hh_l0.shape[1]
+        if H % 128 != 0 or self._emit_mats() is None:
+            return None
+        return (ops.subsampled_length(x.shape[1], 5, 4, 3), x.shape[0], self.encoder.subsample.weight.shape[0], H, lstm.num_layers)
+
+    def _emit_mats(self):
+        L = self.encoder.lstm.num_layers
+        names = (f'encoder.lstm.weight_hh_l{L - 2}', f'encoder.lstm.weight_hh_l{L - 1}', f'encoder.lstm.weight_ih_l{L - 1}')
+        slot = {n: (p, o) for n, p, o in self.flat.slots}
+        return [slot[n] for n in names] if all(n in slot for n in names) else None
+
+    def _emit_versions(self):
+        return (self.flat.params._version,) + tuple(p._version for p, _ in self._emit_mats())
+
+    def _emit_drop(self):
+        if self._graph_emit:
+            self._graphs, self._graph_emit = None, False
+        self._emit = None
+
+    def weights_changed(self):
+        if self._emit is not None:
+            self._emit['current'] = False
+
+    def _emit_begin(self, x, tg):
+        replay = bool(self.use_graph and self._graphs is not None and self._static[0].shape == x.shape and self._static[2].shape == tg.shape)
+        if replay:
+            self._emit_on = self._graph_emit
+        else:
+            key = self._emit_key(x)
+            if self._emit is not None and (key is None or self._emit['key'] != key):
+                self._emit_drop()
+            if key is not None and self._emit is None:
+                reserve = ops.lstm_reserve(*key, self.device)
+                ptrs = ops.lstm_persist2_image_ptrs(reserve, *key)
+                if ptrs is not None:
+                    self._emit = {'key': key, 'reserve': reserve, 'fwd': ptrs[0], 'tr': ptrs[1], 'current': False, 'versions': None,
+                                  'offsets': [o for _, o in self._emit_mats()]}
+            self._emit_on = key is not None and self._emit is not None
+        if self._emit_on:
+            st = self._emit
+            if not st['current'] or st['versions'] != self._emit_versions():
+                w = [p for p, _ in self._emit_mats()]
+                ops.lstm_persist2_pack_images(w[0], w[1], w[2], st['reserve'], *st['key'])
+            st['current'] = False
+
+    def _emit_end(self):
+        if self._emit is not None:
+            self._emit['current'] = self._emit_on
+            self._emit['versions'] = self._emit_versions()
+            if not self._emit_on and not self._graph_emit:
+                self._emit_drop()
 
     def _sharded_tail(self):
         sh = self.sharded
@@ -464,6 +541,7 @@
                 self.sharded.gather_bf16 = False
                 self._tail_graph, self._tail_calls = None, 0
             return self._sharded_step(x, input_lengths, targets, target_lengths)
+        self._emit_begin(x, targets)
         if not self.use_graph:
             st = self._forward_backward_top(x, input_lengths, targets, target_lengths)
             w1 = self.avg_early.start()
@@ -472,8 +550,10 @@
             self.avg_early.finish(w1)
             self.avg_late.finish(w2)
             self._optimizer()
-            return self.loss
-        return self._graph_step(x, input_lengths, targets, target_lengths)
+        else:
+            self._graph_step(x, input_lengths, targets, target_lengths)
+        self._emit_end()
+        return self.loss
 
     def _forward_backward_overlapped(self, x, il, tg, tl):
         sh = self.sharded
@@ -580,6 +660,7 @@
                     self._forward_backward(sx, sil, stg, stl)
                     self._optimizer()
                 self._graphs = (g,)
+                self._graph_emit = self._emit_on
             else:
                 g1, g2, g3 = torch.cuda.CUDAGraph(), torch.cuda.CUDAGraph(), torch.cuda.CUDAGraph()
                 torch.cuda.synchronize()
diff --git a/include/halo.h b/include/halo.h
--- a/include/halo.h
+++ b/include/halo.h
@@ -8,7 +8,7 @@
 extern "C" {
 #endif
 
-#define HALO_ABI_VERSION 19
+#define HALO_ABI_VERSION 20
 
 #define HALO_OK 0
 #define HALO_EINVAL (-22)
@@ -161,6 +161,12 @@
 int halo_lstm_bwd_mid_event_recorded(void);
 int halo_set_lstm_weights_stamp(uint64_t stamp);
 int halo_set_lstm_expect_backward(int on);
+int halo_lstm_persist2_image_ptrs(float *reserve, int T, int B, int in0, int H, int L, void **fwd_images, void **tr_images);
+int halo_lstm_persist2_pack_images(const float *w_hh_lo, const float *w_hh_hi, const float *w_ih_hi, float *reserve, int T, int B, int in0,
+                                   int H, int L, halo_stream_t stream);
+int halo_set_lstm_images_current(const float *reserve, const float *w_hh_lo, const float *w_hh_hi, const float *w_ih_hi, int T, int B,
+                                 int in0, int H, int L);
+int halo_lstm_persist2_last_tile_blocks(void);
 int halo_set_lstm_dx_slabs(int n);
 int halo_lstm_dx_slabs_left(void);
 int halo_set_defer_small_jobs(int on);
@@ -400,6 +406,11 @@
                           const float *weight_decay, const float *const *grad_scale, float lr, const float *lr_dev, float beta1,
                           float beta2, float eps, const uint32_t *step_dev, uint32_t *counter, halo_stream_t stream);
 
+int halo_adamw_ranges_emit_dev(float *p, const float *g, float *m, float *v, int n_ranges, const size_t *begin, const size_t *end,
+                               const float *weight_decay, const float *const *grad_scale, float lr, const float *lr_dev, float beta1,
+                               float beta2, float eps, const uint32_t *step_dev, uint32_t *counter, int n_mats, const size_t *mat_offset,
+                               int H, void *const *fwd_images, void *const *tr_images, halo_stream_t stream);
+
 size_t halo_adamw_multi_tensor_bytes(void);
 unsigned halo_adamw_multi_chunk(void);
 int halo_adamw_multi_max_tensors(void);
```
